# hdm0922/PathTracerDemo

Hardware: AMD Instinct MI355X
Metric: Msamples/sec at 1920x1080, 1 spp ReSTIR DI; per-pixel L2 vs WebGPU ref (higher is better)
Workload: dtype f32; 1 GPU; c3_interior_32 reuse 1920x1080, 1 spp/frame (configs[2]); frame=1920x1080, band_rows_per_gpu=1080, parallelism=row-bands x1

## Files before the change

pathtracerdemo_amd/csrc/ptx_api.cpp:

```cpp
#include <hip/hip_runtime.h>

#include <algorithm>
#include <cmath>
#include <cstdarg>
#include <cstdlib>
#include <cstdio>
#include <cstring>
#include <new>
#include <string>
#include <unordered_map>
#include <vector>

#include "ptx_internal.h"

namespace ptx {


[[maybe_unused]] static const char *const kShippedKnobs[] = {"COMM_TIMEOUT_S", "DEBUG_FILL", "HALO_PROXY_US"};
#if defined(PTX_WG_TIMES)
static const char *const kBuildKind = "wgt";
#elif defined(PTX_AB_BUILD)
static const char *const kBuildKind = "ab";
#else
static const char *const kBuildKind = "product";
// ... 439 lines not shown
                for (int k = 0; k < 3; ++k) P[v][k] = as_f32(G[vi + k]);
            }
            const float e1[3] = {P[1][0] - P[0][0], P[1][1] - P[0][1], P[1][2] - P[0][2]};
            const float e2[3] = {P[2][0] - P[0][0], P[2][1] - P[0][1], P[2][2] - P[0][2]};
            const float rec[12] = {P[0][0], P[0][1], P[0][2], e1[0], e1[1], e1[2], e2[0], e2[1], e2[2], 0, 0, 0};
            tris.insert(tris.end(), rec, rec + 12);
            float N[3][3];
            for (int v = 0; v < 3; ++v) {
                const size_t vi = (size_t)off_vertex + STRIDE_VERTEX * G[ii + v];
                if (vi + 6 > G.size()) return fail(h, PTX_E_SCENE, "vertex normal out of range");
                for (int k = 0; k < 3; ++k) N[v][k] = as_f32(G[vi + 3 + k]);
            }
            const float tv[20] = {P[0][0], P[0][1], P[0][2], N[0][0], N[0][1], N[0][2], P[1][0], P[1][1], P[1][2], N[1][0],
                                  N[1][1], N[1][2], P[2][0], P[2][1], P[2][2], N[2][0], N[2][1], N[2][2], 0.0f, 0.0f};
            tverts.insert(tverts.end(), tv, tv + 20);
        }
    }
    if (tris.empty()) tris.resize(12, 0.0f);
    if (tverts.empty()) tverts.resize(20, 0.0f);
    if (nodes.empty()) nodes.resize(1);
    if (subs.empty()) subs.resize(1);
    h->lay_subs = std::move(subs);
    h->lay_mat_word = std::move(mat_word);
    h->lay_mesh_sub_base = std::move(mesh_sub_base);
    h->lay_mesh_nsub = std::move(mesh_nsub);
    h->lay_mesh_tri_base = std::move(mesh_tri_base);
    h->lay_mesh_ntris = std::move(mesh_ntris);
    h->lay_mesh_vertex = std::move(mesh_vertex);
    h->lay_mesh_nverts = std::move(mesh_nverts);
    h->lay_mesh_node_base = std::move(mesh_node_base);
    h->lay_mesh_nnodes = std::move(mesh_nnodes);
    h->lay_mesh_levels = std::move(mesh_levels);
    h->lay_pair_words = std::move(pair_words);
    h->lay_root_word = std::move(root_word);
    if (int rc = upload(h, h->d_refit_order, order.data(), order.size() * sizeof(uint32_t))) return rc;
    {
        uint32_t most = 1;
        for (const uint32_t t : h->lay_mesh_ntris) most = std::max(most, t);
        if (int rc = alloc_buf(h, h->d_refit_box, (size_t)most * 6u * sizeof(float))) return rc;
    }
    h->n_inst = n_inst;
    if (int rc = layout_tables(h, true, true)) return rc;
    if (int rc = upload(h, h->d_tris, tris.data(), tris.size() * sizeof(float))) return rc;
    if (int rc = upload(h, h->d_nodes, nodes.data(), nodes.size() * sizeof(NodePair))) return rc;
    if (int rc = upload(h, h->d_tverts, tverts.data(), tverts.size() * sizeof(float))) return rc;
    h->n_tris = (uint32_t)(tris.size() / 12);
    h->n_nodes = (uint32_t)nodes.size();
    h->max_depth = max_depth;
    h->stack_depth = max_depth + 2u;
    if ((size_t)h->stack_depth * kBlock * 4u > 160u * 1024u)
        return fail(h, PTX_E_SCENE, "BLAS depth %u needs more LDS than a CU has", max_depth);
    h->layout_valid = true;
    h->layout_gen += 1u;
    for (auto &c : h->ctx) c.surf_valid = false;
    gbuf_key_drop_all(h);
    return PTX_OK;
}

Scene make_scene(ptx_handle *h) {
    Scene sc{};
    std::memcpy(sc.U, h->uniform, sizeof sc.U);
    sc.S = (const uint32_t *)h->d_scene.p;
    sc.G = (const uint32_t *)h->d_geometry.p;
    sc.tris = (const float4 *)h->d_tris.p;
    sc.nodes = (const NodePair *)h->d_nodes.p;
    sc.subs = (const SubRoot *)h->d_subs.p;
    sc.insts = (const Inst *)h->d_insts.p;
    sc.mats = (const float4 *)h->d_mats.p;
    sc.tverts = (const float4 *)h->d_tverts.p;
    sc.lights = sc.S ? sc.S + sc.U[U_OFF_LIGHT] : nullptr;
    sc.cdf = sc.S ? sc.S + sc.U[U_OFF_CDF] : nullptr;
    sc.n_inst = h->n_inst;
    sc.cull_box = h->cull_box;
    sc.cull_pad = h->cull_pad;
    sc.cull_scale = h->cull_scale;
    sc.n_subs = h->n_subs;
    sc.width = h->cfg.width;
    sc.height = h->cfg.height;
    sc.row_begin = h->cfg.row_begin;
    sc.row_end = h->cfg.row_end;
    sc.counters = (h->cfg.flags & PTX_FLAG_COUNT_WORK) ? (unsigned long long *)h->d_counters.p : nullptr;
    sc.census = (h->cfg.flags & PTX_FLAG_ROW_CENSUS) ? (unsigned long long *)h->d_census.p : nullptr;
    sc.frame_color = (float4 *)h->d_frame_color.p;
#ifdef PTX_WG_TIMES
    sc.wgt = (unsigned long long *)h->d_wgt.p;
#endif
    return sc;
}

void resolve_event(TimedLaunch &t, ptx_handle *h) {
    if (!t.pending) return;
    float ms = 0.0f;
    if (hipEventSynchronize(t.stop) == hipSuccess && hipEventElapsedTime(&ms, t.start, t.stop) == hipSuccess) {
        h->ms_total[t.pass] += ms;
        h->launches[t.pass] += 1;
    }
    t.pending = false;
}

static uint32_t seg_pixels(const ptx_handle *h) {
    static const uint32_t env_px = (uint32_t)ab_knob("SEG_PX", 0);
    if (env_px >= 256u && env_px <= 8192u && env_px % 256u == 0u) return env_px;
    const size_t npx = (size_t)h->band_h * h->cfg.width;
    if ((h->cfg.pipeline == PTX_PIPELINE_RESTIR && restir_pipe()) || (h->cfg.pipeline == PTX_PIPELINE_MCPT && mcpt_pipe()) ||
        h->cfg.pipeline == PTX_PIPELINE_RESTIR_GI) {
        const size_t p = (npx / 1152u + 128u) / 256u * 256u;
        return (uint32_t)std::min<size_t>(4096u, std::max<size_t>(kWaveSegPixels, p));
    }
    if (h->cfg.pipeline != PTX_PIPELINE_RESTIR_REUSE) return kWaveSegPixels;
    uint32_t p = 512u;
    while (p < 4096u && (size_t)(2u * p) * 1500u <= npx) p *= 2u;
    return p;
}

static size_t reuse_jobs_per_px(const ptx_handle *h) { return std::max<size_t>(2u * h->reuse_neighbors, kMotionJobs); }
int wave_buffers(ptx_handle *h, WaveBufs &w) {
    const size_t npix = (size_t)h->band_h * h->cfg.width;
    const uint32_t nl = h->uniform[U_LIGHT_COUNT];
    const size_t jpp = !has_reuse(h) ? 1u : h->cfg.pipeline == PTX_PIPELINE_RESTIR_GI ? 2u * h->reuse_neighbors
                                                                                         : reuse_jobs_per_px(h);
    const size_t per_px = std::max<size_t>(std::max<size_t>(2u, (size_t)nl + 1u), jpp);
    const size_t padded = (size_t)((h->cfg.width + 7u) / 8u) * ((h->band_h + 7u) / 8u) * 64u;
    const uint32_t seg_px = seg_pixels(h);
    const size_t nseg = (padded + seg_px - 1u) / seg_px;
    const size_t slots = nseg + 1u;
    const size_t cap = per_px * seg_px * slots;
    const size_t state_b = (size_t)kWaveStateSlots * npix * 16u, act_b = slots * seg_px * jpp * 4u;
    const size_t ctr_b = 2u * kWaveMaxRounds * slots * 4u;
    auto &c = h->cur();
    const bool resize = (c.wstate.p && c.wstate.bytes != state_b) || (c.wact[0].p && c.wact[0].bytes != act_b) ||
                        (c.wact[1].p && c.wact[1].bytes != act_b) || (c.wctr.p && c.wctr.bytes != ctr_b) ||
                        (c.wave_ray_cap && cap > c.wave_ray_cap);
    if (resize)
        if (int rc = quiesce(h)) return rc;
    if (int rc = alloc_buf(h, c.wstate, state_b)) return rc;
    if (int rc = alloc_buf(h, c.wact[0], act_b)) return rc;
    if (int rc = alloc_buf(h, c.wact[1], act_b)) return rc;
    const void *ctr_before = c.wctr.p;
    if (int rc = alloc_buf(h, c.wctr, ctr_b)) return rc;
    if (c.wctr.p != ctr_before) HIP_CHECK(h, memset_sync(h, c.wctr.p, 0, c.wctr.bytes));
    if (h->cfg.pipeline == PTX_PIPELINE_RESTIR_REUSE) {
        const size_t rp_b = slots * (1u + (size_t)seg_px) * 4u;
        if (h->d_replay.p && h->d_replay.bytes != rp_b && !resize)
            if (int rc = quiesce(h)) return rc;
        const void *rp_before = h->d_replay.p;
        if (int rc = alloc_buf(h, h->d_replay, rp_b)) return rc;
        if (h->d_replay.p != rp_before) HIP_CHECK(h, memset_sync(h, h->d_replay.p, 0, slots * 4u));
    }
    if (cap > c.wave_ray_cap) {
        free_buf(c.wrays);
        for (DevBuf &r : c.wres) free_buf(r);
        c.wave_ray_cap = 0;
        if (int rc = alloc_buf(h, c.wrays, cap * 32u)) return rc;
        for (int i = 0; i < (h->cfg.pipeline == PTX_PIPELINE_RESTIR_REUSE ? 3 : 2); ++i)
            if (int rc = alloc_buf(h, c.wres[i], cap * 32u)) return rc;
        c.wave_ray_cap = cap;
    }
    w.surf = nullptr;
    if (h->cfg.pipeline == PTX_PIPELINE_RESTIR_REUSE) {
        const size_t rows = (size_t)h->halo_top + h->band_h + h->halo_bot;
        if (c.surf.bytes != rows * h->cfg.width * 32u) c.surf_valid = false;
        if (int rc = alloc_buf(h, c.surf, rows * h->cfg.width * 32u)) return rc;
        w.surf = (uint4 *)c.surf.p + 2u * (size_t)h->halo_top * h->cfg.width;
    }
    w.state = (float4 *)c.wstate.p;
    w.npix = (uint32_t)npix;
    w.seg_px = seg_px;
    w.nseg = (uint32_t)nseg;
    w.ray_stride = (uint32_t)(per_px * seg_px);
    w.rays = (float4 *)c.wrays.p;
    for (int i = 0; i < 3; ++i) w.res[i] = (float4 *)c.wres[i].p;
    w.nres = 2;
    for (int i = 0; i < 2; ++i) w.act[i] = (uint32_t *)c.wact[i].p;
    w.act_stride = (uint32_t)(seg_px * jpp);
    w.cnt = (uint32_t *)c.wctr.p;
    w.seg_base = 0;
    w.seg_count = w.nseg;
    static const uint32_t cl = (uint32_t)ab_knob("SEG_CLUSTER", 1);
    w.cluster = (cl == 2u || cl == 4u || cl == 8u || cl == 16u) ? cl : 1u;
    if (h->cfg.flags & PTX_FLAG_ROW_CENSUS) w.cluster = seg_px / 64u;
    w.tile0 = 0;
    w.ntile0 = (uint32_t)(padded / 64u);
    w.tile1 = w.ntile1 = 0;
    w.seg_phys = 0;
    w.cnt_stride = (uint32_t)slots;
    return PTX_OK;
}

static TimedLaunch *event_begin(ptx_handle *h, int slot, hipStream_t st) {
    if (!(h->cfg.flags & PTX_FLAG_TIME_LAUNCHES)) return nullptr;
    TimedLaunch &t = h->ring[h->ring_pos];
    h->ring_pos = (h->ring_pos + 1) % kEventRing;
    resolve_event(t, h);
    if (hipEventRecord(t.start, st) != hipSuccess) return nullptr;
    t.pass = slot;
    return &t;
}
static void event_end(TimedLaunch *t, hipStream_t st) {
    if (t && hipEventRecord(t->stop, st) == hipSuccess) t->pending = true;
}

static size_t px_with_halo(const ptx_handle *h) {
    return (size_t)(h->halo_top + h->band_h + h->halo_bot) * h->cfg.width;
}
static uint32_t gi_job_slots(const ptx_handle *h) { return std::max(2u * h->reuse_neighbors, kGiMotionSlots); }
int reuse_buffers(ptx_handle *h) {
    const size_t njobs = (size_t)h->band_h * h->cfg.width *
                         (h->cfg.pipeline == PTX_PIPELINE_RESTIR_GI ? gi_job_slots(h) : reuse_jobs_per_px(h));
    if (h->cfg.pipeline == PTX_PIPELINE_RESTIR_GI) return alloc_buf(h, h->d_jres, njobs * 4u);
    if (int rc = alloc_buf(h, h->d_jstate, njobs * 6u * 16u)) return rc;
    if (int rc = alloc_buf(h, h->cur().nbr, px_with_halo(h) * 16u)) return rc;
    const size_t npix = (size_t)h->band_h * h->cfg.width;
    if (int rc = alloc_buf(h, h->cur().tjstate, npix * kMotionJobs * 6u * 16u)) return rc;
    if (int rc = alloc_buf(h, h->cur().tjres, npix * kMotionJobs * 16u)) return rc;
    return alloc_buf(h, h->d_jres, njobs * 16u);
}
static ReuseArgs reuse_args(ptx_handle *h, int pass) {
    ReuseArgs A{};
    A.gbuf = gbuf_band(h);
    A.cur = res_band(h);
    A.hist = hist_band(h);
    const bool temporal = pass == PTX_PASS_TEMPORAL;
    A.jstate = (float4 *)(temporal ? h->cur().tjstate.p : h->d_jstate.p);
    A.jres = (float4 *)(temporal ? h->cur().tjres.p : h->d_jres.p);
    A.jpp = temporal ? 1u : 2u * h->reuse_neighbors;
    A.njobs = h->band_h * h->cfg.width * A.jpp;
    static const bool planes = ab_knob("JOB_PLANES", 1) != 0;
    A.jpx = planes ? 1u : A.jpp;
    A.jslot = planes ? h->band_h * h->cfg.width : 1u;
    A.radius = h->reuse_radius;
    A.neighbors = h->reuse_neighbors;
    A.cap = h->temporal_cap;
    A.hist_valid = h->hist_valid && !h->hist_moved ? 1u : 0u;
    A.use_init = (pass == PTX_PASS_TEMPORAL && h->cur().init_state_valid) ? 1u : 0u;
    A.nbr_out = (uint4 *)h->cur().nbr.p + (size_t)h->halo_top * h->cfg.width;
    A.nbr = A.nbr_out;
    A.surf = h->cur().surf.p ? (const uint4 *)h->cur().surf.p + 2u * (size_t)h->halo_top * h->cfg.width : nullptr;
    static const bool fold_off = ab_knob("FOLD_LAST_STEP", 1) == 0;
    A.fold_last = ((pass == PTX_PASS_SPATIAL || pass == PTX_PASS_TEMPORAL) && !fold_off) ? 1u : 0u;
    A.ray_cap = (uint32_t)std::min<size_t>(h->cur().wave_ray_cap, 0xffffffffu);
    return A;
}

void mat4_inverse(const float *mf, float *out);
static ReuseArgs motion_args(ptx_handle *h) {
    ReuseArgs A = reuse_args(h, PTX_PASS_SPATIAL);
    A.jstate = (float4 *)h->cur().tjstate.p;
    A.jres = (float4 *)h->cur().tjres.p;
    A.jpp = kMotionJobs;
    A.njobs = h->band_h * h->cfg.width * A.jpp;
    static const bool planes = ab_knob("JOB_PLANES", 1) != 0;
    A.jpx = planes ? 1u : A.jpp;
    A.jslot = planes ? h->band_h * h->cfg.width : 1u;
    A.hist_valid = h->hist_valid ? 1u : 0u;
    A.use_init = h->cur().init_state_valid ? 1u : 0u;
    static const bool fold_on = ab_knob("FOLD_LAST_STEP", 1) != 0;
    A.fold_last = fold_on ? 1u : 0u;
    A.motion = 1u;
    std::memcpy(A.vpinv_prev, h->hist_camera, sizeof A.vpinv_prev);
    mat4_inverse(A.vpinv_prev, A.vp_prev);
    const size_t W = h->cfg.width;
    A.psurf = (const uint4 *)h->d_psurf.p + 2u * (size_t)h->halo_top * W;
    A.prev_row_lo = -(int32_t)h->halo_top;
    A.prev_row_hi = (int32_t)(h->band_h + h->halo_bot);
    A.clip = (unsigned long long *)h->d_counters.p + CNT_MOTION_CLIP;
    return A;
}

static GiArgs gi_args(ptx_handle *h, bool motion) {
    GiArgs A{};
    A.gbuf = gbuf_band(h);
    A.cur = res_band(h);
    A.hist = hist_band(h);
    A.direct = (float4 *)h->cur().direct.p;
    A.accum = (float4 *)h->d_accum.p;
    A.jray = (uint32_t *)h->d_jres.p;
    A.jpp = 2u * h->reuse_neighbors;
    static const bool planes = ab_knob("GI_JOB_PLANES", 1) != 0;
    A.jpx = planes ? 1u : A.jpp;
    A.jslot = planes ? h->band_h * h->cfg.width : 1u;
    if (!planes && motion) A.jpx = gi_job_slots(h);
    A.radius = h->reuse_radius;
    A.neighbors = h->reuse_neighbors;
    A.cap = h->temporal_cap;
    A.hist_valid = h->hist_valid && (motion || !h->hist_moved) ? 1u : 0u;
    if (motion) {
        std::memcpy(A.vpinv_prev, h->hist_camera, sizeof A.vpinv_prev);
        mat4_inverse(A.vpinv_prev, A.vp_prev);
        A.pgbuf = (const uint4 *)h->d_psurf.p + (size_t)h->halo_top * h->cfg.width;
        A.prev_row_lo = -(int32_t)h->halo_top;
        A.prev_row_hi = (int32_t)(h->band_h + h->halo_bot);
        A.clip = (unsigned long long *)h->d_counters.p + CNT_MOTION_CLIP;
    }
    return A;
}

static bool fuse_spatial_final(const ptx_handle *h, const Scene &sc, const int *passes, int npasses, int i) {
    static const bool on = ab_knob("FINAL_ONE", 1) != 0;
    return on && i + 1 < npasses && passes[i] == PTX_PASS_SPATIAL && passes[i + 1] == PTX_PASS_FINAL &&
           h->cfg.pipeline == PTX_PIPELINE_RESTIR_REUSE && tables_fit_lds(sc) && h->d_replay.p;
}

static hipError_t launch_wave_seq(ptx_handle *h, const Scene &sc, const WaveBufs &w, int pass, hipStream_t st,
                                  bool fused = false, hipEvent_t combine_after = nullptr,
                                  hipEvent_t combine_done = nullptr) {
    const uint4 *gb = gbuf_band(h);
    uint4 *res = res_band(h);
    float4 *acc = (float4 *)h->d_accum.p;
    hipError_t e = hipSuccess;
    if (h->cfg.pipeline == PTX_PIPELINE_RESTIR_GI) {
        const bool motion = is_motion_pass(pass);
        const GiArgs A = gi_args(h, motion);
        const int gp = motion ? 4 : pass == PTX_PASS_INIT ? 0 : pass == PTX_PASS_TEMPORAL ? 1 : pass == PTX_PASS_SPATIAL ? 2 : 3;
        const int rounds = gp == 0 ? kWaveRoundsGiInit : gp == 2 || gp == 4 ? kWaveRoundsGiSpatial : 0;
        for (int r = 0; e == hipSuccess && r <= rounds; ++r) {
            if (r > 0) {
                TimedLaunch *t = event_begin(h, PTX_STAT_WAVE_TRACE, st);
                e = wave_trace(sc, w, r - 1, 1, h->stack_depth, st, gp >= 2);
                event_end(t, st);
                if (e != hipSuccess) break;
            }
            TimedLaunch *t = event_begin(h, PTX_STAT_WAVE_LOGIC, st);
            e = wave_gi_round(sc, w, gp, r, A, st);
            event_end(t, st);
        }
        return e;
    }
    if (pass == PTX_PASS_TEMPORAL || pass == PTX_PASS_SPATIAL || pass == kPassTemporalJobs ||
        pass == kPassTemporalCombine || is_motion_pass(pass)) {
        const bool temporal = pass != PTX_PASS_SPATIAL;
        ReuseArgs A = is_motion_pass(pass) ? motion_args(h)
                                           : reuse_args(h, temporal ? PTX_PASS_TEMPORAL : PTX_PASS_SPATIAL);
        WaveBufs wj = w;
        if (A.fold_last && wj.res[2]) wj.nres = 3;
        else A.fold_last = 0u;
        if (fused && pass == PTX_PASS_SPATIAL) {
            A.fuse_final = 1u;
            A.accum = (float4 *)h->d_accum.p;
            A.replay_cnt = (uint32_t *)h->d_replay.p;
            A.replay = A.replay_cnt + w.cnt_stride;
            A.replay_total = (unsigned long long *)h->d_counters.p + CNT_REPLAY;
        }
        const int nr = reuse_rounds(temporal, A);
        const int r_first = pass == kPassTemporalCombine ? nr + 1 : 0;
        const int r_last = pass == kPassTemporalJobs ? nr : nr + 1;
        for (int r = r_first; e == hipSuccess && r <= r_last; ++r) {
            if (r > 0 && r <= nr) {
                TimedLaunch *t = event_begin(h, PTX_STAT_WAVE_TRACE, st);
                e = wave_trace(sc, wj, r - 1, 1, h->stack_depth, st);
                event_end(t, st);
            }
            if (e != hipSuccess) break;
            if (r == nr && A.fold_last) continue;
            const bool combine = r == nr + 1 && pass == PTX_PASS_SPATIAL;
            if (combine && combine_after && (e = hipStreamWaitEvent(st, combine_after, 0)) != hipSuccess) break;
            TimedLaunch *t = event_begin(h, PTX_STAT_WAVE_LOGIC, st);
            e = wave_reuse_round(sc, wj, temporal, r, A, st);
            event_end(t, st);
            if (combine && combine_done && e == hipSuccess) e = hipEventRecord(combine_done, st);
        }
        return e;
    }
    const uint4 *fres = h->cfg.pipeline == PTX_PIPELINE_RESTIR_REUSE ? (const uint4 *)hist_band(h) : res;
    static const bool final_one = ab_knob("FINAL_ONE", 1) != 0;
    if (pass == PTX_PASS_FINAL && final_one && h->cfg.pipeline == PTX_PIPELINE_RESTIR_REUSE && tables_fit_lds(sc)) {
        TimedLaunch *t = event_begin(h, PTX_STAT_WAVE_LOGIC, st);
        if (fused)
            e = wave_final_replay(sc, w, gb, fres, acc, (const uint32_t *)h->d_replay.p + w.cnt_stride,
                                  (uint32_t *)h->d_replay.p, h->stack_depth, st);
        else
            e = wave_final_one(sc, w, gb, fres, acc, h->stack_depth, st);
        event_end(t, st);
        h->launches[PTX_STAT_FINAL_FUSED] += 1;
        h->cur().init_state_valid = false;
        return e;
    }
    h->cur().init_state_valid = pass == PTX_PASS_INIT && h->cfg.pipeline == PTX_PIPELINE_RESTIR_REUSE;
    const int rounds = pass == PTX_PASS_INIT ? kWaveRoundsInit : pass == PTX_PASS_FINAL ? kWaveRoundsFinal
                                                                                        : kWaveRoundsMcpt;
    for (int r = 0; e == hipSuccess && r <= rounds; ++r) {
        if (r > 0) {
            TimedLaunch *t = event_begin(h, PTX_STAT_WAVE_TRACE, st);
            e = wave_trace(sc, w, r - 1, 1, h->stack_depth, st);
            event_end(t, st);
        }
        if (e != hipSuccess) break;
        TimedLaunch *t = event_begin(h, PTX_STAT_WAVE_LOGIC, st);
        e = pass == PTX_PASS_INIT    ? wave_init_round(sc, w, r, gb, res, st)
            : pass == PTX_PASS_FINAL ? wave_final_round(sc, w, r, gb, fres, acc, st)
                                     : wave_mcpt_round(sc, w, r, acc, h->mcpt_color, st);
        event_end(t, st);
    }
    return e;
}

hipError_t spatial_summaries(ptx_handle *h, hipStream_t st) {
    if (h->cfg.pipeline != PTX_PIPELINE_RESTIR_REUSE) return hipSuccess;
    const size_t W = h->cfg.width, top = h->halo_top * W, band = (size_t)h->band_h * W;
    const uint4 *gb = (const uint4 *)h->cur().gbuf.p, *rs = (const uint4 *)h->cur().res.p;
    uint4 *nb = (uint4 *)h->cur().nbr.p, *sf = (uint4 *)h->cur().surf.p;
    const Scene sc = make_scene(h);
    TimedLaunch *t = event_begin(h, PTX_STAT_WAVE_LOGIC, st);
    hipError_t e;
    if (!h->cur().nbr_valid) {
        e = wave_reuse_summary(sc, gb, rs, nb, sf, px_with_halo(h), st);
    } else {
        e = top ? wave_reuse_summary(sc, gb, rs, nb, sf, top, st) : hipSuccess;
        const size_t b0 = top + band;
        if (e == hipSuccess && px_with_halo(h) > b0)
            e = wave_reuse_summary(sc, gb + b0, rs + 8u * b0, nb + b0, sf ? sf + 2u * b0 : nullptr, px_with_halo(h) - b0,
                                   st);
    }
    event_end(t, st);
    return e;
}

static bool frames_in_flight(const ptx_handle *h) { return h->ctx[1].own && pipelined(h); }
static hipError_t fork_sequences(ptx_handle *h, int k) {
    auto &c = h->cur();
    hipError_t e = hipSuccess;
    if (k <= 1) return e;
    if (!c.ev_fork && (e = hipEventCreateWithFlags(&c.ev_fork, hipEventDisableTiming)) != hipSuccess) return e;
    for (int q = 1; q < k; ++q) {
        if (!c.sub[q] && (e = hipStreamCreateWithFlags(&c.sub[q], hipStreamNonBlocking)) != hipSuccess) return e;
        if (!c.ev_join[q] && (e = hipEventCreateWithFlags(&c.ev_join[q], hipEventDisableTiming)) != hipSuccess) return e;
    }
    if ((e = hipEventRecord(c.ev_fork, c.stream)) != hipSuccess) return e;
    for (int q = 1; q < k && e == hipSuccess; ++q) e = hipStreamWaitEvent(c.sub[q], c.ev_fork, 0);
    return e;
}
static hipError_t join_sequences(ptx_handle *h, int k) {
    auto &c = h->cur();
    hipError_t e = hipSuccess;
    for (int q = 1; q < k && e == hipSuccess; ++q)
        if ((e = hipEventRecord(c.ev_join[q], c.sub[q])) == hipSuccess) e = hipStreamWaitEvent(c.stream, c.ev_join[q], 0);
    return e;
}

static void seg_share(WaveBufs &part, uint32_t nseg, int q, int k) {
    part.seg_base = (uint32_t)((uint64_t)nseg * q / k);
    part.seg_count = (uint32_t)((uint64_t)nseg * (q + 1) / k) - part.seg_base;
}
static hipError_t spatial_overlap_seq(ptx_handle *h, const Scene &sc, const WaveBufs &interior, const WaveBufs &edge,
                                      hipEvent_t halo) {
    hipError_t e = hipSuccess;
    static const int env_bk = ab_knob("PIPE_BACK_STREAMS", 2);
    int k = env_bk > 0 && frames_in_flight(h) ? env_bk : 1;
    if (h->cfg.flags & PTX_FLAG_SINGLE_STREAM) k = 1;
    k = std::max(1, std::min<int>({k, ptx_handle::kMaxSplit, (int)interior.nseg, (int)edge.nseg}));
    ReuseArgs A = reuse_args(h, PTX_PASS_SPATIAL);
    const bool fold = A.fold_last && interior.res[2];
    if (!fold) A.fold_last = 0u;
    const int nr = reuse_rounds(0, A);
    if ((e = fork_sequences(h, k)) != hipSuccess) return e;
    const bool surf_stale = interior.surf && !h->cur().surf_valid;
    uint32_t E = 0u;
    for (int q = 0; q < k && e == hipSuccess; ++q) {
        hipStream_t st = q ? h->cur().sub[q] : h->cur().stream;
        WaveBufs wi = interior, we = edge;
        seg_share(wi, interior.nseg, q, k);
        seg_share(we, edge.nseg, q, k);
        wi.seg_phys = interior.seg_phys + E;
        we.seg_phys = interior.seg_phys + E + wi.seg_base + wi.seg_count - we.seg_base;
        E += we.seg_count;
        if (fold) wi.nres = we.nres = 3;
        WaveBufs wt = wi;
        wt.seg_count = wi.seg_count + we.seg_count;
        if (surf_stale) {
            if ((e = wave_surface(sc, wi, gbuf_band(h), st)) != hipSuccess) return e;
            if ((e = wave_surface(sc, we, gbuf_band(h), st)) != hipSuccess) return e;
        }
        for (int r = 0; e == hipSuccess && r <= nr + 1; ++r) {
            if (r > 0 && r <= nr) {
                TimedLaunch *t = event_begin(h, PTX_STAT_WAVE_TRACE, st);
                e = wave_trace(sc, wt, r - 1, 1, h->stack_depth, st);
                event_end(t, st);
                if (e != hipSuccess) break;
            }
            if (r == nr && A.fold_last) continue;
            TimedLaunch *t = event_begin(h, PTX_STAT_WAVE_LOGIC, st);
            e = wave_reuse_round(sc, wi, 0, r, A, st);
            if (e == hipSuccess && r == 0 && halo) e = hipStreamWaitEvent(st, halo, 0);
            if (e == hipSuccess) e = wave_reuse_round(sc, we, 0, r, A, st);
            event_end(t, st);
        }
        for (const WaveBufs *ws : {&wi, &we})
            if (e == hipSuccess) e = launch_wave_seq(h, sc, *ws, PTX_PASS_FINAL, st);
    }
    if (surf_stale && e == hipSuccess) h->cur().surf_valid = true;
    return e == hipSuccess ? join_sequences(h, k) : e;
}

hipError_t launch_wave_parts(ptx_handle *h, const Scene &sc, const WaveBufs &w, const int *passes, int npasses,
                             bool summaries, const WaveBufs *then, hipEvent_t then_wait, bool keep_gbuf) {
    h->hand_n = 0;
    static const bool overlap_start = ab_knob("OVERLAP_START", 1) != 0;
    if (then && overlap_start && npasses == 2 && passes[0] == PTX_PASS_SPATIAL && passes[1] == PTX_PASS_FINAL &&
        h->cfg.pipeline == PTX_PIPELINE_RESTIR_REUSE && !summaries)
        return spatial_overlap_seq(h, sc, w, *then, then_wait);
    static const int env_k = ab_knob("WAVE_STREAMS", 0);
    static const int env_pk = ab_knob("PIPE_STREAMS", 0);
    const bool band_h = h->comm || h->halo_top || h->halo_bot || (h->cfg.flags & PTX_FLAG_HALO_SKIP);
    const int pipe_k = env_pk > 0 ? env_pk : band_h || h->cfg.pipeline == PTX_PIPELINE_RESTIR_GI ? 1 : 2;
    int k = frames_in_flight(h) ? pipe_k : env_k > 0 ? env_k : 3;
    static const int env_bk = ab_knob("PIPE_BACK_STREAMS", 2);
    if (env_bk > 0 && frames_in_flight(h))
        for (int i = 0; i < npasses; ++i)
            if (passes[i] == PTX_PASS_SPATIAL) k = env_bk;
    if (h->cfg.flags & PTX_FLAG_SINGLE_STREAM) k = 1;
    k = std::max(1, std::min<int>(k, ptx_handle::kMaxSplit));
    if ((uint32_t)k > std::max(w.nseg, then ? then->nseg : 0u)) k = (int)std::max(w.nseg, then ? then->nseg : 0u);
    hipError_t e = hipSuccess;
    bool has_gbuf = false;
    for (int i = 0; i < npasses; ++i) has_gbuf |= passes[i] == PTX_PASS_GBUFFER;
    const bool skip_gbuf = has_gbuf && keep_gbuf && gbuf_kept(h);
    if (has_gbuf && !skip_gbuf) h->cur().gbuf_key_valid = false;
    for (int i = 0; i < npasses; ++i) {
        if (passes[i] == PTX_PASS_SPATIAL) {
            if (summaries && (e = spatial_summaries(h, h->cur().stream)) != hipSuccess) return e;
        } else if (passes[i] == PTX_PASS_GBUFFER && skip_gbuf) {
            continue;
        } else if (passes[i] != PTX_PASS_FINAL && passes[i] != PTX_PASS_TEMPORAL && passes[i] != kPassTemporalJobs &&
                   passes[i] != kPassTemporalCombine && !is_motion_pass(passes[i])) {
            h->cur().nbr_valid = false;
        }
    }
    bool need_surf[8] = {false};
    bool surf_ok = h->cur().surf_valid;
    for (int i = 0; i < npasses && i < 8; ++i) {
        if (passes[i] == PTX_PASS_GBUFFER) surf_ok = surf_ok && skip_gbuf;
        else if (passes[i] == PTX_PASS_INIT && w.surf) surf_ok = true;
        else if ((passes[i] == PTX_PASS_TEMPORAL || passes[i] == kPassTemporalJobs || passes[i] == PTX_PASS_SPATIAL ||
                  is_motion_pass(passes[i])) &&
                 w.surf) {
            need_surf[i] = !surf_ok;
            surf_ok = true;
        }
    }
    h->cur().surf_valid = surf_ok && w.surf;
    if (k == 0) return hipSuccess;
    if ((e = fork_sequences(h, k)) != hipSuccess) return e;
    for (int q = 0; q < k; ++q) {
        hipStream_t st = q ? h->cur().sub[q] : h->cur().stream;
        for (int set = 0; set < (then ? 2 : 1); ++set) {
            const WaveBufs &ws = set ? *then : w;
            if (set && then_wait && (e = hipStreamWaitEvent(st, then_wait, 0)) != hipSuccess) return e;
            WaveBufs part = ws;
            seg_share(part, ws.nseg, q, k);
            if (!part.seg_count) continue;
            for (int i = 0; i < npasses; ++i) {
                if (passes[i] == PTX_PASS_GBUFFER) {
                    if (skip_gbuf) continue;
                    TimedLaunch *t = event_begin(h, PTX_PASS_GBUFFER, st);
                    e = wave_gbuffer(sc, part, gbuf_band(h), h->stack_depth, st);
                    h->cur().init_state_valid = false;
                    event_end(t, st);
                } else {
                    if (i < 8 && need_surf[i]) {
                        TimedLaunch *t = event_begin(h, PTX_STAT_WAVE_LOGIC, st);
                        e = wave_surface(sc, part, gbuf_band(h), st);
                        event_end(t, st);
                        if (e != hipSuccess) return e;
                    }
                    const bool fused = !then && (fuse_spatial_final(h, sc, passes, npasses, i) ||
                                                 (i > 0 && fuse_spatial_final(h, sc, passes, npasses, i - 1)));
                    e = launch_wave_seq(h, sc, part, passes[i], st, fused);
                }
                if (e != hipSuccess) return e;
            }
        }
    }
    if ((e = join_sequences(h, k)) != hipSuccess) return e;
    if (has_gbuf && !skip_gbuf) {
        gbuf_key_of(h, h->cur().gbuf_key);
        h->cur().gbuf_key_valid = true;
    }
    for (int i = 0; i < npasses; ++i)
        if (passes[i] == PTX_PASS_TEMPORAL || passes[i] == kPassTemporalCombine || passes[i] == kPassTemporalMotion) {
            h->cur().init_state_valid = false;
            h->cur().nbr_valid = h->cfg.pipeline == PTX_PIPELINE_RESTIR_REUSE;
        }
    return hipSuccess;
}
static hipError_t launch_wave_pass(ptx_handle *h, const Scene &sc, const WaveBufs &w, int pass) {
    return launch_wave_parts(h, sc, w, &pass, 1);
}

static hipError_t launch_back_chain(ptx_handle *h, const Scene &sc, const WaveBufs &w, bool with_temporal,
                                    const hipEvent_t *hand, int n_hand) {
    auto &c = h->cur();
    if (h->comm || h->halo_top || h->halo_bot || (h->cfg.flags & PTX_FLAG_HALO_SKIP) || !w.surf || !c.surf_valid ||
        (!with_temporal && !c.nbr_valid))
        return hipErrorNotSupported;
    static const int env_bk = ab_knob("PIPE_BACK_STREAMS", 2);
    const int k = std::max(1, std::min<int>({env_bk > 0 ? env_bk : 1, ptx_handle::kMaxSplit, (int)w.nseg}));
    hipError_t e = hipSuccess;
    for (int q = 0; q < k; ++q) {
        if (!c.ev_tc[q] && (e = hipEventCreateWithFlags(&c.ev_tc[q], hipEventDisableTiming)) != hipSuccess) return e;
        if (!c.ev_hand[q] && (e = hipEventCreateWithFlags(&c.ev_hand[q], hipEventDisableTiming)) != hipSuccess) return e;
    }
    if ((e = fork_sequences(h, k)) != hipSuccess) return e;
    WaveBufs part[ptx_handle::kMaxSplit];
    for (int q = 0; q < k; ++q) {
        part[q] = w;
        seg_share(part[q], w.nseg, q, k);
    }
    for (int q = 0; q < k && with_temporal; ++q) {
        hipStream_t st = q ? c.sub[q] : c.stream;
        for (int i = 0; i < n_hand; ++i)
            if ((e = hipStreamWaitEvent(st, hand[i], 0)) != hipSuccess) return e;
        if (n_hand == 0 && (e = hipStreamWaitEvent(st, h->ev_prev, 0)) != hipSuccess) return e;
        if (part[q].seg_count && (e = launch_wave_seq(h, sc, part[q], kPassTemporalCombine, st)) != hipSuccess) return e;
        if ((e = hipEventRecord(c.ev_tc[q], st)) != hipSuccess) return e;
    }
    if (with_temporal) {
        c.init_state_valid = false;
        c.nbr_valid = true;
    }
// ... 1285 lines not shown
        reuse |= passes[i] == PTX_PASS_TEMPORAL || passes[i] == PTX_PASS_SPATIAL;
    }
    const uint32_t fl = h->cfg.flags;
    if (fl & (PTX_FLAG_SIMPLE_KERNELS | PTX_FLAG_COUNT_WORK)) {
        for (int i = 0; i < n; ++i)
            if (int rc = timed_launch(h, passes[i])) return rc;
        h->rendered = true;
        h->drawn |= gb;
        return PTX_OK;
    }
    if (!h->scene_loaded || !h->frame_set) return fail(h, PTX_E_INVALID, "scene and frame must be set before rendering");
    if (!h->layout_valid) {
        if (int rc = build_layout(h)) return rc;
    }
    Scene sc = make_scene(h);
    if (gb && !tables_fit_lds(sc)) {
        for (int i = 0; i < n; ++i)
            if (int rc = timed_launch(h, passes[i])) return rc;
        h->rendered = true;
        h->drawn |= gb;
        return PTX_OK;
    }
    WaveBufs w{};
    if (int rc = wave_buffers(h, w)) return rc;
    if (reuse)
        if (int rc = reuse_buffers(h)) return rc;
    TimedLaunch &t = h->ring[h->ring_pos];
    h->ring_pos = (h->ring_pos + 1) % kEventRing;
    resolve_event(t, h);
    HIP_CHECK(h, hipEventRecord(t.start, h->cur().stream));
    const hipError_t e = launch_wave_parts(h, sc, w, passes, n);
    if (e != hipSuccess) return fail(h, PTX_E_HIP, "ptx_run_passes: %s", hipGetErrorString(e));
    HIP_CHECK(h, hipEventRecord(t.stop, h->cur().stream));
    t.pass = PTX_STAT_PASS_GROUP;
    t.pending = true;
    for (int i = 0; i < n; ++i)
        if (passes[i] == PTX_PASS_SPATIAL) mark_history(h);
    h->rendered = true;
    h->drawn |= gb;
    return PTX_OK;
}

int ptx_halo_rows(ptx_handle *h, uint32_t *rows_top, uint32_t *rows_bottom, size_t *bytes_per_row) {
    if (!h) return PTX_E_INVALID;
    if (rows_top) *rows_top = h->halo_top;
    if (rows_bottom) *rows_bottom = h->halo_bot;
    if (bytes_per_row) *bytes_per_row = (size_t)h->cfg.width * (16u + 16u * h->res_u4);
    return PTX_OK;
}

static int halo_copy(ptx_handle *h, uint32_t r0, uint32_t rows, void *msg, bool to_msg) {
    if (!rows) return PTX_OK;
    const size_t W = h->cfg.width, rpx = 16u * h->res_u4, gb = rows * W * 16u, rb = rows * W * rpx;
    char *g = (char *)h->cur().gbuf.p + (size_t)r0 * W * 16u, *r = (char *)h->cur().res.p + (size_t)r0 * W * rpx;
    char *m = (char *)msg;
    if (to_msg) {
        HIP_CHECK(h, hipMemcpyAsync(m, g, gb, hipMemcpyDefault, h->cur().stream));
        HIP_CHECK(h, hipMemcpyAsync(m + gb, r, rb, hipMemcpyDefault, h->cur().stream));
    } else {
        gbuf_key_drop(h);
        HIP_CHECK(h, hipMemcpyAsync(g, m, gb, hipMemcpyDefault, h->cur().stream));
        HIP_CHECK(h, hipMemcpyAsync(r, m + gb, rb, hipMemcpyDefault, h->cur().stream));
    }
    return PTX_OK;
}

int ptx_halo_pack(ptx_handle *h, void *dev_top, void *dev_bottom) {
    if (!h) return PTX_E_INVALID;
    if ((h->halo_top && !dev_top) || (h->halo_bot && !dev_bottom)) return fail(h, PTX_E_INVALID, "ptx_halo_pack: null buffer");
    if (int rc = halo_copy(h, h->halo_top, h->halo_top, dev_top, true)) return rc;
    return halo_copy(h, h->halo_top + h->band_h - h->halo_bot, h->halo_bot, dev_bottom, true);
}

int ptx_halo_unpack(ptx_handle *h, const void *dev_top, const void *dev_bottom) {
    if (!h) return PTX_E_INVALID;
    if ((h->halo_top && !dev_top) || (h->halo_bot && !dev_bottom)) return fail(h, PTX_E_INVALID, "ptx_halo_unpack: null buffer");
    if (int rc = halo_copy(h, 0u, h->halo_top, (void *)dev_top, false)) return rc;
    return halo_copy(h, h->halo_top + h->band_h, h->halo_bot, (void *)dev_bottom, false);
}

int ptx_render(ptx_handle *h, float *rgba_out) {
    if (!h) return PTX_E_INVALID;
    HIP_CHECK(h, hipSetDevice(h->device));
    if (h->cfg.pipeline == PTX_PIPELINE_RESTIR) {
        int rc = timed_wave_frame(h);
        if (rc < 0) return rc;
        if (rc == 1)
            for (int p : {PTX_PASS_GBUFFER, PTX_PASS_INIT, PTX_PASS_FINAL})
                if ((rc = timed_launch(h, p))) return rc;
    } else if (has_reuse(h) && h->comm) {
        if (int rc = render_band_nccl(h)) return rc;
        if (rgba_out)
            if (int rc = read_to_host(h, rgba_out, h->d_accum.p, h->d_accum.bytes)) return rc;
        return PTX_OK;
    } else if (has_reuse(h) && (h->halo_top || h->halo_bot) && (h->cfg.flags & PTX_FLAG_HALO_SKIP)) {
        if (int rc = render_band_solo(h)) return rc;
        if (rgba_out)
            if (int rc = read_to_host(h, rgba_out, h->d_accum.p, h->d_accum.bytes)) return rc;
        return PTX_OK;
    } else if (has_reuse(h)) {
        if (h->halo_top || h->halo_bot)
            return fail(h, PTX_E_INVALID, "a band of the reuse pipeline renders with a communicator "
                                          "(ptx_comm_init), through ptx_render_bands, or ptx_run_passes + ptx_halo_*");
        int rc = timed_wave_frame(h);
        if (rc < 0) return rc;
        if (rc == 1)
            for (int p : {PTX_PASS_GBUFFER, PTX_PASS_INIT, PTX_PASS_TEMPORAL, PTX_PASS_SPATIAL, PTX_PASS_FINAL})
                if ((rc = timed_launch(h, p))) return rc;
    } else if (pipelined(h)) {
        int rc = timed_wave_frame(h);
        if (rc < 0) return rc;
        if (rc == 1 && (rc = timed_launch(h, PTX_PASS_MCPT))) return rc;
    } else {
        if (int rc = timed_launch(h, PTX_PASS_MCPT)) return rc;
    }
    h->frames++;
    h->rendered = h->drawn = true;
    if (rgba_out)
        if (int rc = read_to_host(h, rgba_out, h->d_accum.p, h->d_accum.bytes)) return rc;
    return PTX_OK;
}

int ptx_reset_accumulation(ptx_handle *h) {
    if (!h) return PTX_E_INVALID;
    HIP_CHECK(h, hipMemsetAsync(h->d_accum.p, 0, h->d_accum.bytes, h->cur().stream));
    h->hist_valid = false;
    h->dn_hist_valid = false;
    h->ut_valid = false;
    return PTX_OK;
}

int ptx_synchronize(ptx_handle *h) {
    if (!h) return PTX_E_INVALID;
    HIP_CHECK(h, hipStreamSynchronize(h->cur().stream));
    return PTX_OK;
}

int ptx_get_stats(ptx_handle *h, ptx_stats *out) {
    if (!h || !out) return PTX_E_INVALID;
    for (auto &t : h->ring) resolve_event(t, h);
    std::memset(out, 0, sizeof *out);
    out->frames = h->frames;
    for (int p = 0; p < kPasses; ++p) {
        out->kernel_ms_total[p] = h->ms_total[p];
        out->kernel_launches[p] = h->launches[p];
    }
    out->triangles = h->n_tris;
    out->bvh_nodes = h->n_nodes;
    out->instances = h->n_inst;
    out->max_bvh_depth = h->max_depth;
    const auto &c = h->cur();
    out->device_bytes = h->d_scene.bytes + h->d_geometry.bytes + h->d_tris.bytes + h->d_nodes.bytes + h->d_subs.bytes +
                        h->d_insts.bytes + h->d_mats.bytes + h->d_tverts.bytes + c.gbuf.bytes + c.res.bytes + h->d_accum.bytes +
                        h->d_hist.bytes + h->d_jstate.bytes + h->d_jres.bytes + c.tjstate.bytes + c.tjres.bytes + c.nbr.bytes +
                        c.surf.bytes + h->d_psurf.bytes + c.direct.bytes + h->d_dn_guide.bytes + h->d_dn_work.bytes +
                        h->d_denoised.bytes + h->d_frame_color.bytes + h->d_dn_guide_prev.bytes + h->d_dn_hist[0].bytes +
                        h->d_dn_hist[1].bytes + h->d_dn_mom[0].bytes + h->d_dn_mom[1].bytes + h->d_dn_halo_g.bytes +
                        h->d_dn_halo_c.bytes + h->d_dn_obj.bytes + h->d_dn_snap.bytes + h->d_up_halo.bytes + h->d_ut_guide[0].bytes + h->d_ut_guide[1].bytes +
                        h->d_ut_hist[0].bytes + h->d_ut_hist[1].bytes + h->d_refit_order.bytes + h->d_refit_box.bytes;
    for (const auto &k : h->skins) out->device_bytes += k.bind.bytes + k.target_pos.bytes + k.target_nrm.bytes + k.pose.bytes;
    return PTX_OK;
}

int ptx_reset_stats(ptx_handle *h) {
    if (!h) return PTX_E_INVALID;
    for (auto &t : h->ring) t.pending = false;
    HIP_CHECK(h, hipStreamSynchronize(h->cur().stream));
    for (int p = 0; p < kPasses; ++p) { h->ms_total[p] = 0.0; h->launches[p] = 0; }
    h->frames = 0;
    HIP_CHECK(h, memset_sync(h, h->d_counters.p, 0, h->d_counters.bytes));
    if (h->d_census.p) HIP_CHECK(h, memset_sync(h, h->d_census.p, 0, h->d_census.bytes));
    return PTX_OK;
}

#ifdef PTX_WG_TIMES
int ptx_diag_wave_times(ptx_handle *h, uint64_t *out, size_t max_records) {
    if (!h || !h->d_wgt.p) return PTX_E_INVALID;
    HIP_CHECK(h, hipDeviceSynchronize());
    uint64_t n = 0;
    HIP_CHECK(h, copy_sync(h, &n, h->d_wgt.p, 8, hipMemcpyDeviceToHost));
    n = std::min<uint64_t>(std::min<uint64_t>(n, 1u << 20), max_records);
    if (n && out) HIP_CHECK(h, copy_sync(h, out, (uint64_t *)h->d_wgt.p + 4, n * 32u, hipMemcpyDeviceToHost));
    HIP_CHECK(h, memset_sync(h, h->d_wgt.p, 0, 8));
    return (int)n;
}
#endif

int ptx_row_census(ptx_handle *h, uint64_t *out, size_t n_tile_rows) {
    if (!h || !out) return PTX_E_INVALID;
    if (!(h->cfg.flags & PTX_FLAG_ROW_CENSUS)) return fail(h, PTX_E_INVALID, "handle has no PTX_FLAG_ROW_CENSUS");
    const uint32_t tile_rows = (h->band_h + 7u) / 8u, tiles_x = (h->cfg.width + 7u) / 8u;
    if (n_tile_rows != tile_rows) return fail(h, PTX_E_INVALID, "census: %zu tile rows, band has %u", n_tile_rows, tile_rows);
    std::vector<unsigned long long> c((size_t)h->census_blocks * kCensusWords);
    HIP_CHECK(h, copy_sync(h, c.data(), h->d_census.p, c.size() * 8u, hipMemcpyDeviceToHost));
    std::memset(out, 0, (size_t)tile_rows * 5u * sizeof(uint64_t));
    for (uint32_t r = 0; r < tile_rows; ++r)
        for (int k = 0; k < 5; ++k) out[5u * r + k] += c[(size_t)kCensusWords * r + k];
    const uint32_t m = seg_pixels(h) / 64u, ntiles = tile_rows * tiles_x;
    for (uint32_t s = 0; tile_rows + s < h->census_blocks && (size_t)s * m < ntiles; ++s) {
        const unsigned long long *b = c.data() + (size_t)kCensusWords * (tile_rows + s);
        const uint32_t t0 = s * m, t1 = std::min(ntiles, t0 + m), r0 = t0 / tiles_x, r1 = (t1 - 1u) / tiles_x;
        for (int k = 0; k < 5; ++k) {
            uint64_t left = b[k];
            for (uint32_t r = r0; r <= r1; ++r) {
                const uint32_t a = std::max(t0, r * tiles_x), z = std::min(t1, (r + 1u) * tiles_x);
                const uint64_t part = r == r1 ? left : b[k] * (z - a) / (t1 - t0);
                out[5u * r + k] += part;
                left -= part;
            }
        }
    }
    return PTX_OK;
}

int ptx_read_buffer(ptx_handle *h, int which, void *host_dst, size_t bytes) {
    if (!h || !host_dst) return PTX_E_INVALID;
    DevBuf b;
    if (!buffer_view(h, which, b) || bytes > b.bytes)
        return fail(h, PTX_E_INVALID, "read of %zu bytes from buffer %d", bytes, which);
    if (int rc = read_to_host(h, host_dst, b.p, bytes)) return rc;
    return PTX_OK;
}

int ptx_write_buffer(ptx_handle *h, int which, const void *host_src, size_t bytes) {
    if (!h || !host_src) return PTX_E_INVALID;
    DevBuf b;
    if (which == PTX_BUF_DENOISED) return fail(h, PTX_E_INVALID, "the denoised image is ptx_denoise's output: read-only");
    if (which == PTX_BUF_FRAME_COLOR || which == PTX_BUF_DENOISE_HISTORY)
        return fail(h, PTX_E_INVALID, "buffer %d is the renderer's / ptx_denoise's output: read-only", which);
    if (which == PTX_BUF_UPSAMPLE_HISTORY)
        return fail(h, PTX_E_INVALID, "buffer %d is ptx_upsample_temporal's output: read-only", which);
    if (!buffer_view(h, which, b) || bytes > b.bytes)
        return fail(h, PTX_E_INVALID, "write of %zu bytes to buffer %d", bytes, which);
    HIP_CHECK(h, copy_sync(h, b.p, host_src, bytes, hipMemcpyHostToDevice));
    h->cur().init_state_valid = false;
    h->cur().nbr_valid = false;
    h->cur().surf_valid = false;
    if (which == PTX_BUF_GBUFFER) gbuf_key_drop(h);
    return PTX_OK;
}

int ptx_device_pointer(ptx_handle *h, int which, void **dev_ptr, size_t *bytes) {
    if (!h || !dev_ptr) return PTX_E_INVALID;
    DevBuf b;
    if (!buffer_view(h, which, b)) return fail(h, PTX_E_INVALID, "unknown buffer %d", which);
    *dev_ptr = b.p;
    if (bytes) *bytes = b.bytes;
    if (which == PTX_BUF_GBUFFER) {
        h->gbuf_exposed = true;
        gbuf_key_drop_all(h);
    }
    return PTX_OK;
}

int ptx_present(ptx_handle *h, uint32_t canvas_w, uint32_t canvas_h, int bgra, uint8_t *out) {
    if (!h || !out) return PTX_E_INVALID;
    if (canvas_w == 0 || canvas_h == 0 || (uint64_t)canvas_w * canvas_h > (1ull << 28))
        return fail(h, PTX_E_INVALID, "ptx_present: canvas %ux%u", canvas_w, canvas_h);
    if (h->cfg.row_begin != 0 || h->band_h != h->cfg.height)
        return fail(h, PTX_E_INVALID, "ptx_present: a band handle (rows %u..%u) holds part of the texture: present the "
                                      "gathered frame on the host", h->cfg.row_begin, h->cfg.row_end);
    if (!h->d_accum.p) return fail(h, PTX_E_INVALID, "ptx_present: nothing rendered");
    HIP_CHECK(h, hipSetDevice(h->device));
    const size_t bytes = (size_t)canvas_w * canvas_h * 4u;
    if (int rc = alloc_buf(h, h->d_canvas, bytes)) return rc;
    const hipError_t e = launch_present(present_texture(h), h->cfg.width, h->cfg.height, canvas_w, canvas_h,
                                        bgra != 0, (uint32_t *)h->d_canvas.p, h->cur().stream);
    if (e != hipSuccess) return fail(h, PTX_E_HIP, "ptx_present: %s", hipGetErrorString(e));
    return read_to_host(h, out, h->d_canvas.p, bytes);
}

int ptx_present_async(ptx_handle *h, uint32_t canvas_w, uint32_t canvas_h, int bgra) {
    if (!h) return PTX_E_INVALID;
    if (h->present_pending) return fail(h, PTX_E_INVALID, "ptx_present_async: a present is in flight (poll it first)");
    if (canvas_w == 0 || canvas_h == 0 || (uint64_t)canvas_w * canvas_h > (1ull << 28))
        return fail(h, PTX_E_INVALID, "ptx_present_async: canvas %ux%u", canvas_w, canvas_h);
    if (h->cfg.row_begin != 0 || h->band_h != h->cfg.height)
        return fail(h, PTX_E_INVALID, "ptx_present_async: a band handle holds part of the texture");
    if (!h->d_accum.p) return fail(h, PTX_E_INVALID, "ptx_present_async: nothing rendered");
    HIP_CHECK(h, hipSetDevice(h->device));
    const size_t bytes = (size_t)canvas_w * canvas_h * 4u;
    if (int rc = alloc_buf(h, h->d_canvas_async, bytes)) return rc;
    if (bytes > h->present_host_bytes) {
        if (h->present_host) (void)hipHostFree(h->present_host);
        h->present_host = nullptr;
        h->present_host_bytes = 0;
        HIP_CHECK(h, hipHostMalloc(&h->present_host, bytes, hipHostMallocDefault));
        h->present_host_bytes = bytes;
    }
    if (!h->ev_present) HIP_CHECK(h, hipEventCreateWithFlags(&h->ev_present, hipEventDisableTiming));
    const hipError_t e = launch_present(present_texture(h), h->cfg.width, h->cfg.height, canvas_w, canvas_h,
                                        bgra != 0, (uint32_t *)h->d_canvas_async.p, h->cur().stream);
    if (e != hipSuccess) return fail(h, PTX_E_HIP, "ptx_present_async: %s", hipGetErrorString(e));
    HIP_CHECK(h, hipMemcpyAsync(h->present_host, h->d_canvas_async.p, bytes, hipMemcpyDeviceToHost, h->cur().stream));
    HIP_CHECK(h, hipEventRecord(h->ev_present, h->cur().stream));
    h->present_bytes = bytes;
    h->present_pending = true;
    return PTX_OK;
}

int ptx_present_poll(ptx_handle *h, uint8_t *out, size_t bytes) {
    if (!h || !out) return PTX_E_INVALID;
    if (!h->present_pending) return fail(h, PTX_E_INVALID, "ptx_present_poll: no present in flight");
    if (bytes < h->present_bytes)
        return fail(h, PTX_E_INVALID, "ptx_present_poll: %zu bytes; the canvas needs %zu", bytes, h->present_bytes);
    const hipError_t e = hipEventQuery(h->ev_present);
    if (e == hipErrorNotReady) return PTX_E_PENDING;
// ... 24 lines not shown
int ptx_upsample(ptx_handle *hi, ptx_handle *lo, const ptx_upsample_params *p) {
    if (!hi || !lo) return PTX_E_INVALID;
    const char *what = "ptx_upsample";
    if (hi == lo) return fail(hi, PTX_E_INVALID, "%s: one handle on both sides", what);
    float sigma_plane;
    if (int rc = upsample_params(hi, p, sigma_plane, what)) return rc;
    for (ptx_handle *h : {hi, lo})
        if (h->cfg.row_begin != 0 || h->band_h != h->cfg.height)
            return fail(hi, PTX_E_INVALID, "%s: the %s handle is a band (rows %u..%u): ptx_upsample_bands", what,
                        h == hi ? "full-size" : "small", h->cfg.row_begin, h->cfg.row_end);
    uint32_t s = 0;
    if (int rc = upsample_pair_check(hi, hi, lo, s, what)) return rc;
    HIP_CHECK(hi, hipSetDevice(hi->device));
    if (int rc = upsample_alloc(hi, 0u, lo->cfg.width)) return rc;
    if (int rc = upsample_source(hi, lo)) return rc;
    HIP_CHECK(hi, hipStreamWaitEvent(hi->cur().stream, lo->ev_up_src, 0));
    const hipError_t e = upsample_launch(hi, lo, s, sigma_plane, 0u, 0u);
    if (int rc = upsample_done(hi, hi)) return rc;
    if (int rc = upsample_release(hi, lo, hi)) return rc;
    if (e != hipSuccess) return fail(hi, PTX_E_HIP, "%s launch: %s", what, hipGetErrorString(e));
    return PTX_OK;
}

int ptx_phase_uniform(const uint32_t hi_uniform[PTX_UNIFORM_WORDS], uint32_t s, uint32_t px, uint32_t py,
                      uint32_t lo_uniform_out[PTX_UNIFORM_WORDS]) {
    if (!hi_uniform || !lo_uniform_out) return PTX_E_INVALID;
    if (s < 2u || s > 4u || px >= s || py >= s) return PTX_E_INVALID;
    const uint32_t W = hi_uniform[0], H = hi_uniform[1];
    if (W == 0u || H == 0u || W % s != 0u || H % s != 0u) return PTX_E_INVALID;
    uint32_t u[PTX_UNIFORM_WORDS];
    std::memcpy(u, hi_uniform, sizeof u);
    u[0] = W / s;
    u[1] = H / s;
    const float dx = (float)(2 * (int)px - ((int)s - 1)) / (float)W, dy = (float)(2 * (int)py - ((int)s - 1)) / (float)H;
    if (dx != 0.0f || dy != 0.0f) {
#pragma clang fp contract(off)
        float m[16];
        std::memcpy(m, u + 4, sizeof m);
        for (int k = 0; k < 4; ++k) {
            const float a = dx * m[k], b = dy * m[4 + k];
            const float t = m[12 + k] + a;
            m[12 + k] = t + b;
        }
        std::memcpy(u + 4, m, sizeof m);
    }
    std::memcpy(lo_uniform_out, u, sizeof u);
    return PTX_OK;
}

int ptx_upsample_temporal(ptx_handle *hi, ptx_handle *lo, const ptx_upsample_temporal_params *p) {
    if (!hi || !lo) return PTX_E_INVALID;
    const char *what = "ptx_upsample_temporal";
    if (hi == lo) return fail(hi, PTX_E_INVALID, "%s: one handle on both sides", what);
    UtCall c;
    if (int rc = upsample_temporal_params(hi, p, c, what, false)) return rc;
    for (ptx_handle *h : {hi, lo})
        if (h->cfg.row_begin != 0 || h->band_h != h->cfg.height)
            return fail(hi, PTX_E_INVALID, "%s: the %s handle is a band (rows %u..%u): bands are not supported by this call", what,
                        h == hi ? "full-size" : "small", h->cfg.row_begin, h->cfg.row_end);
    uint32_t s = 0;
    if (int rc = upsample_pair_check(hi, hi, lo, s, what, false)) return rc;
    if (int rc = upsample_temporal_camera(hi, hi, lo, s, c, what)) return rc;
    HIP_CHECK(hi, hipSetDevice(hi->device));
    if (int rc = upsample_temporal_alloc(hi, hi, 0u, lo->cfg.width)) return rc;
    if (int rc = upsample_source(hi, lo)) return rc;
    HIP_CHECK(hi, hipStreamWaitEvent(hi->cur().stream, lo->ev_up_src, 0));
    const hipError_t e = upsample_temporal_launch(hi, lo, s, c, 0u, 0u, 0u, 0u);
    if (int rc = upsample_done(hi, hi)) return rc;
    if (int rc = upsample_release(hi, lo, hi)) return rc;
    if (e != hipSuccess) return fail(hi, PTX_E_HIP, "%s launch: %s", what, hipGetErrorString(e));
    return PTX_OK;
}

int ptx_present_source(ptx_handle *h, int which) {
    if (!h) return PTX_E_INVALID;
    if (which != PTX_BUF_ACCUM && which != PTX_BUF_DENOISED)
        return fail(h, PTX_E_INVALID, "ptx_present_source: buffer %d (PTX_BUF_ACCUM or PTX_BUF_DENOISED)", which);
    if (which == PTX_BUF_DENOISED && !h->d_denoised.p)
        return fail(h, PTX_E_INVALID, "ptx_present_source: no denoised image yet (ptx_denoise first)");
    h->present_src = which;
    return PTX_OK;
}

int ptx_trace_device(ptx_handle *h, const void *rays_dev, void *hits_dev, size_t n, int eps_mode) {
    if (!h || (n && (!rays_dev || !hits_dev)) || n > 0xffffffffu || (eps_mode != 0 && eps_mode != 1))
        return fail(h, PTX_E_INVALID, "ptx_trace: bad arguments");
    if (!h->scene_loaded || !h->frame_set) return fail(h, PTX_E_INVALID, "scene and frame must be set before tracing");
    if (!h->layout_valid) {
        if (int rc = build_layout(h)) return rc;
    }
    TimedLaunch &t = h->ring[h->ring_pos];
    h->ring_pos = (h->ring_pos + 1) % kEventRing;
    resolve_event(t, h);
    Scene sc = make_scene(h);
    HIP_CHECK(h, hipEventRecord(t.start, h->cur().stream));
    const bool simple = (h->cfg.flags & PTX_FLAG_SIMPLE_KERNELS) != 0;
    hipError_t e = (simple ? launch_trace_rays : launch_trace_rays_sm)(
        sc, (const float4 *)rays_dev, (float4 *)hits_dev, (uint32_t)n, eps_mode, h->stack_depth, h->cur().stream);
    if (e != hipSuccess) return fail(h, PTX_E_HIP, "trace launch: %s", hipGetErrorString(e));
    HIP_CHECK(h, hipEventRecord(t.stop, h->cur().stream));
    t.pass = PTX_PASS_TRACE;
    t.pending = true;
    return PTX_OK;
}

int ptx_trace(ptx_handle *h, const float *rays, float *hits, size_t n, int eps_mode) {
    if (!h || (n && (!rays || !hits))) return fail(h, PTX_E_INVALID, "ptx_trace: null arrays");
    if (n == 0) return PTX_OK;
    if (int rc = alloc_buf(h, h->d_qrays, std::max(h->d_qrays.bytes, n * 32u))) return rc;
    if (int rc = alloc_buf(h, h->d_qhits, std::max(h->d_qhits.bytes, n * 32u))) return rc;
    HIP_CHECK(h, hipMemcpyAsync(h->d_qrays.p, rays, n * 32u, hipMemcpyHostToDevice, h->cur().stream));
    if (int rc = ptx_trace_device(h, h->d_qrays.p, h->d_qhits.p, n, eps_mode)) return rc;
    return read_to_host(h, hits, h->d_qhits.p, n * 32u);
}

int ptx_trace_queries(ptx_handle *h, const float *queries, float *results, size_t n, int eps_mode, int occ_only) {
    if (!h || (n && (!queries || !results))) return fail(h, PTX_E_INVALID, "ptx_trace_queries: null arrays");
    if (eps_mode != 0 && eps_mode != 1) return fail(h, PTX_E_INVALID, "ptx_trace_queries: eps_mode %d (0 or 1)", eps_mode);
    if (h->cfg.flags & (PTX_FLAG_SIMPLE_KERNELS | PTX_FLAG_ROW_CENSUS))
        return fail(h, PTX_E_INVALID, "ptx_trace_queries: the handle has no wavefront trace kernel of its own "
                                      "(PTX_FLAG_SIMPLE_KERNELS) or maps queue slots to tile rows (PTX_FLAG_ROW_CENSUS)");
    if (!h->scene_loaded || !h->frame_set) return fail(h, PTX_E_INVALID, "scene and frame must be set before tracing");
    if (n > 0x7fffffffu) return fail(h, PTX_E_INVALID, "ptx_trace_queries: %zu queries (32-bit ray slots)", n);
    for (size_t i = 0; i < n; ++i) {
        uint32_t kind;
        std::memcpy(&kind, queries + 8u * i + 7u, sizeof kind);
        if (kind > 2u) return fail(h, PTX_E_INVALID, "ptx_trace_queries: query %zu has kind %u (0 closest, 1 Visibility, 2 occlusion)", i, kind);
        if (occ_only && kind != 2u)
            return fail(h, PTX_E_INVALID, "ptx_trace_queries: occ_only with query %zu of kind %u (every query must be 2, occlusion)", i, kind);
    }
    if (n == 0) return PTX_OK;
    if (!h->layout_valid) {
        if (int rc = build_layout(h)) return rc;
    }
    const uint32_t nseg = (uint32_t)((n + kWaveSegPixels - 1u) / kWaveSegPixels);
    const size_t slots = (size_t)nseg * kWaveSegPixels;
    std::vector<uint32_t> cnt(2u * (size_t)nseg, 0u);
    for (uint32_t j = 0; j < nseg; ++j)
        cnt[nseg + j] = (uint32_t)std::min<size_t>(kWaveSegPixels, n - (size_t)j * kWaveSegPixels);
    if (int rc = alloc_buf(h, h->d_qrays, std::max(h->d_qrays.bytes, slots * 32u))) return rc;
    if (int rc = alloc_buf(h, h->d_qhits, std::max(h->d_qhits.bytes, slots * 32u))) return rc;
    if (int rc = alloc_buf(h, h->d_qcnt, std::max(h->d_qcnt.bytes, cnt.size() * 4u))) return rc;
    hipStream_t st = h->cur().stream;
    HIP_CHECK(h, hipMemcpyAsync(h->d_qrays.p, queries, n * 32u, hipMemcpyHostToDevice, st));
    HIP_CHECK(h, hipMemcpyAsync(h->d_qcnt.p, cnt.data(), cnt.size() * 4u, hipMemcpyHostToDevice, st));
    HIP_CHECK(h, hipMemsetAsync(h->d_qhits.p, 0, n * 32u, st));
    WaveBufs w{};
    w.seg_px = kWaveSegPixels;
    w.nseg = w.seg_count = w.cnt_stride = nseg;
    w.cluster = 1;
    w.ray_stride = kWaveSegPixels;
    w.rays = (float4 *)h->d_qrays.p;
    w.res[0] = w.res[1] = (float4 *)h->d_qhits.p;
    w.nres = 2;
    w.cnt = (uint32_t *)h->d_qcnt.p;
    TimedLaunch &t = h->ring[h->ring_pos];
    h->ring_pos = (h->ring_pos + 1) % kEventRing;
    resolve_event(t, h);
    Scene sc = make_scene(h);
    HIP_CHECK(h, hipEventRecord(t.start, st));
    hipError_t e = wave_trace(sc, w, 0, eps_mode, h->stack_depth, st, occ_only != 0);
    if (e != hipSuccess) return fail(h, PTX_E_HIP, "trace launch: %s", hipGetErrorString(e));
    HIP_CHECK(h, hipEventRecord(t.stop, st));
    t.pass = PTX_PASS_TRACE;
    t.pending = true;
    return read_to_host(h, results, h->d_qhits.p, n * 32u);
}

int ptx_set_stream(ptx_handle *h, void *hip_stream) {
    if (!h) return PTX_E_INVALID;
    if (int rc = first_frame_ctx(h)) return rc;
    if (h->ev_up_src || h->d_denoised.p)
        if (int rc = quiesce(h)) return rc;
    h->ctx[0].stream = hip_stream ? (hipStream_t)hip_stream : h->ctx[0].own;
    h->dn_stream = h->ctx[0].stream;
    gbuf_key_drop_all(h);
    return PTX_OK;
}

int ptx_destroy(ptx_handle *h) {
    if (!h) return PTX_E_INVALID;
    (void)hipSetDevice(h->device);
    (void)quiesce(h);
    if (h->xstream) (void)hipStreamSynchronize(h->xstream);
    comm_destroy(h);
    if (h->ctx[0].own) (void)hipStreamSynchronize(h->ctx[0].own);
    for (auto &t : h->ring) {
        if (t.start) (void)hipEventDestroy(t.start);
        if (t.stop) (void)hipEventDestroy(t.stop);
    }
    if (h->host_stage) (void)hipHostFree(h->host_stage);
    if (h->ev_present) {
        (void)hipEventSynchronize(h->ev_present);
        (void)hipEventDestroy(h->ev_present);
    }
    if (h->present_host) (void)hipHostFree(h->present_host);
    for (DevBuf *b : {&h->d_canvas, &h->d_canvas_async, &h->d_scene, &h->d_geometry, &h->d_tris, &h->d_nodes, &h->d_subs,
                      &h->d_insts, &h->d_mats, &h->d_tverts, &h->d_accum, &h->d_counters, &h->d_qrays, &h->d_qhits, &h->d_qcnt, &h->d_hist,
                      &h->d_jstate, &h->d_jres, &h->d_replay, &h->d_psurf, &h->d_census, &h->d_wgt, &h->d_dn_guide, &h->d_dn_work,
                      &h->d_denoised, &h->d_frame_color, &h->d_dn_guide_prev, &h->d_dn_hist[0], &h->d_dn_hist[1], &h->d_dn_mom[0],
                      &h->d_dn_mom[1], &h->d_dn_halo_g, &h->d_dn_halo_c, &h->d_dn_obj, &h->d_dn_snap, &h->d_up_halo, &h->d_ut_guide[0], &h->d_ut_guide[1],
                      &h->d_ut_hist[0], &h->d_ut_hist[1], &h->d_refit_order, &h->d_refit_box})
        free_buf(*b);
    drop_skins(h);
    for (auto &c : h->ctx) {
        for (DevBuf *b : {&c.gbuf, &c.res, &c.direct, &c.nbr, &c.tjstate, &c.tjres, &c.surf, &c.wstate, &c.wrays, &c.wres[0],
                          &c.wres[1], &c.wres[2], &c.wact[0], &c.wact[1], &c.wctr})
            free_buf(*b);
        if (c.ev_fork) (void)hipEventDestroy(c.ev_fork);
        for (int q = 0; q < ptx_handle::kMaxSplit; ++q) {
            if (c.ev_join[q]) (void)hipEventDestroy(c.ev_join[q]);
            if (c.sub[q]) (void)hipStreamDestroy(c.sub[q]);
        }
        if (c.own) (void)hipStreamDestroy(c.own);
    }
    if (h->ev_prev) (void)hipEventDestroy(h->ev_prev);
    if (h->ev_dn_ready) (void)hipEventDestroy(h->ev_dn_ready);
    if (h->ev_dn_copied) (void)hipEventDestroy(h->ev_dn_copied);
    if (h->ev_up_src) (void)hipEventDestroy(h->ev_up_src);
    if (h->ev_up_done) (void)hipEventDestroy(h->ev_up_done);
    if (h->ev_ut_ready) (void)hipEventDestroy(h->ev_ut_ready);
    if (h->ev_ut_copied) (void)hipEventDestroy(h->ev_ut_copied);
    delete h;
    return PTX_OK;
}

const char *ptx_last_error(const ptx_handle *h) { return h ? h->err.c_str() : "null handle"; }

}
```

pathtracerdemo_amd/csrc/ptx_internal.h:

```cpp
#pragma once
#include <hip/hip_runtime.h>

#include <algorithm>
#include <string>

#include "../../include/ptx.h"
#include "ptx_launch.h"

namespace ptx {
constexpr int kPasses = 16;
constexpr int kEventRing = 256;
struct DevBuf {
    void *p = nullptr;
    size_t bytes = 0;
};
struct TimedLaunch {
    hipEvent_t start = nullptr, stop = nullptr;
    int pass = -1;
    bool pending = false;
};
}

using namespace ptx;

constexpr int kPassTemporalJobs = 0x100, kPassTemporalCombine = 0x101;
constexpr int kPassTemporalMotion = 0x102;
inline bool is_motion_pass(int p) {
    return p == kPassTemporalMotion;
}

constexpr uint8_t kStaleGeometry = 1u, kStaleAccel = 2u;

struct ptx_handle {
    ptx_config cfg{};
    int device = 0;
    std::string err;

    std::vector<uint32_t> scene, geometry, accel;
    DevBuf d_scene, d_geometry;
    DevBuf d_tris, d_nodes, d_subs, d_insts, d_mats, d_tverts;
    uint32_t n_tris = 0, n_nodes = 0, n_inst = 0, n_subs = 0, max_depth = 0, stack_depth = 0;
    float cull_box = 0.0f, cull_pad = 0.0f, cull_scale = 0.0f;
    uint32_t layout_key[8] = {0};
    bool layout_valid = false;
    std::vector<SubRoot> lay_subs;
    std::vector<size_t> lay_mat_word;
    std::vector<uint32_t> lay_mesh_sub_base, lay_mesh_nsub, lay_mesh_tri_base;
    std::vector<uint32_t> lay_mesh_ntris, lay_mesh_vertex, lay_mesh_nverts, lay_mesh_node_base, lay_mesh_nnodes;
    std::vector<std::vector<uint32_t>> lay_mesh_levels;
    std::vector<uint32_t> lay_pair_words, lay_root_word;
    DevBuf d_refit_order, d_refit_box;
    struct Skin {
        uint32_t first = 0, n = 0, n_joints = 0, n_targets = 0;
        double w_max = 0.0, p_max = 0.0, d_max = 0.0;
        DevBuf bind, target_pos, target_nrm, pose;
    };
    std::vector<Skin> skins;
    std::vector<uint8_t> mesh_stale;
    bool scene_loaded = false;
    uint32_t uniform[PTX_UNIFORM_WORDS] = {0};
    bool frame_set = false;
    uint32_t band_h = 0, halo_top = 0, halo_bot = 0;
    DevBuf d_accum, d_counters, d_hist, d_jstate, d_jres;
    DevBuf d_replay;
    uint32_t res_u4 = 8;
    bool gbuf_exposed = false;
    uint32_t reuse_radius = 0, reuse_neighbors = 0, temporal_cap = 0;
    float4 *mcpt_color = nullptr;
    bool hist_valid = false;
    uint32_t hist_camera[19] = {0};
    bool hist_moved = false;
    bool hist_same_only = false;
    DevBuf d_psurf;
    DevBuf d_qrays, d_qhits;
    DevBuf d_qcnt;
    DevBuf d_census;
    uint32_t census_blocks = 0;
    DevBuf d_wgt;
    static constexpr int kMaxCtx = 3;
    static constexpr int kMaxSplit = 4;
    static constexpr int kGbufKeyWords = 32;
    struct FrameCtx {
        DevBuf gbuf, res, direct;
        DevBuf nbr, tjstate, tjres;
        DevBuf surf;
        DevBuf wstate, wrays, wres[3], wact[2], wctr;
        size_t wave_ray_cap = 0;
        hipStream_t own = nullptr, stream = nullptr;
        hipStream_t sub[kMaxSplit] = {nullptr, nullptr, nullptr, nullptr};
        hipEvent_t ev_fork = nullptr, ev_join[kMaxSplit] = {nullptr, nullptr, nullptr, nullptr};
        hipEvent_t ev_tc[kMaxSplit] = {nullptr, nullptr, nullptr, nullptr};
        hipEvent_t ev_hand[kMaxSplit] = {nullptr, nullptr, nullptr, nullptr};
        bool init_state_valid = false;
        bool nbr_valid = false;
        bool surf_valid = false;
        uint32_t gbuf_key[kGbufKeyWords] = {0};
        bool gbuf_key_valid = false;
    } ctx[kMaxCtx];
    int ctx_idx = 0;
    FrameCtx &cur() { return ctx[ctx_idx]; }
    const FrameCtx &cur() const { return ctx[ctx_idx]; }
    hipEvent_t ev_prev = nullptr;
    int hand_ctx = 0, hand_n = 0;
    void *comm = nullptr;
    int rank = 0, world = 1;
    hipStream_t xstream = nullptr;
    hipEvent_t ev_front = nullptr, ev_halo = nullptr;
    hipEvent_t ev_mhalo = nullptr;
    uint64_t halo_bytes_sent = 0;
    bool comm_broken = false;
    uint64_t band_frames = 0;
    uint32_t band_camera[19] = {0};
    DevBuf d_canvas;
    void *host_stage = nullptr;
    size_t host_stage_bytes = 0;
    DevBuf d_canvas_async;
    void *present_host = nullptr;
    size_t present_host_bytes = 0, present_bytes = 0;
    hipEvent_t ev_present = nullptr;
    bool present_pending = false;
    DevBuf d_dn_guide, d_dn_work, d_denoised;
    DevBuf d_frame_color;
    DevBuf d_dn_guide_prev, d_dn_hist[2], d_dn_mom[2];
    int dn_set = 0;
    bool dn_hist_valid = false;
    uint32_t dn_camera[19] = {0};
    float dn_vp[16] = {0};
    std::vector<uint32_t> dn_insts;
    DevBuf d_dn_obj;
    bool dn_track = false;
    uint32_t dn_track_layout = 0, layout_gen = 0;
    DevBuf d_dn_snap;
    std::vector<uint8_t> dn_deformed;
    uint32_t dn_cap_top = 0, dn_cap_bot = 0;
    DevBuf d_dn_halo_g, d_dn_halo_c;
    uint32_t dn_cov_lo = 0, dn_cov_hi = 0;
    hipEvent_t ev_dn_ready = nullptr, ev_dn_copied = nullptr;
    bool dn_guide_swapped = false, drawn = false;
    hipStream_t dn_stream = nullptr;
    hipEvent_t ev_up_src = nullptr, ev_up_done = nullptr;
    uint32_t dn_guide_top = 0, dn_guide_bot = 0;
    DevBuf d_up_halo;
    DevBuf d_ut_guide[2], d_ut_hist[2];
    int ut_set = 0;
    bool ut_valid = false, dn_guide_stale = false;
    uint32_t ut_camera[19] = {0};
    float ut_vp[16] = {0};
    hipEvent_t ev_ut_ready = nullptr, ev_ut_copied = nullptr;
    uint32_t nb_rows[2][2] = {{0, 0}, {0, 0}};
    int present_src = PTX_BUF_ACCUM;
    bool rendered = false;
    TimedLaunch ring[kEventRing];
    int ring_pos = 0;
    double ms_total[kPasses] = {};
    uint64_t launches[kPasses] = {};
    uint64_t frames = 0;
};

namespace ptx {
int fail(ptx_handle *h, int code, const char *fmt, ...);
#define HIP_CHECK(h, expr)                                                                                   \
    do {                                                                                                     \
        hipError_t e_ = (expr);                                                                              \
        if (e_ != hipSuccess) return fail((h), PTX_E_HIP, "%s: %s (%s:%d)", #expr, hipGetErrorString(e_),      \
                                          __FILE__, __LINE__);                                               \
    } while (0)
void free_buf(DevBuf &b);
int alloc_buf(ptx_handle *h, DevBuf &b, size_t bytes);
int read_to_host(ptx_handle *h, void *dst, const void *src, size_t bytes);
uint4 *gbuf_band(ptx_handle *h);
uint4 *res_band(ptx_handle *h);
bool has_reuse(const ptx_handle *h);
int build_layout(ptx_handle *h);
Scene make_scene(ptx_handle *h);
void resolve_event(TimedLaunch &t, ptx_handle *h);
int wave_buffers(ptx_handle *h, WaveBufs &w);
int reuse_buffers(ptx_handle *h);
hipError_t launch_wave_parts(ptx_handle *h, const Scene &sc, const WaveBufs &w, const int *passes, int npasses,
                             bool summaries = true, const WaveBufs *then = nullptr, hipEvent_t then_wait = nullptr,
                             bool keep_gbuf = false);
void gbuf_key_of(const ptx_handle *h, uint32_t *key);
void gbuf_key_drop(ptx_handle *h);
void gbuf_key_drop_all(ptx_handle *h);
hipError_t spatial_summaries(ptx_handle *h, hipStream_t st);
void mark_history(ptx_handle *h);
int motion_prepare(ptx_handle *h, hipStream_t st);
uint4 *hist_band(ptx_handle *h);
bool pipelined(const ptx_handle *h);
int quiesce(ptx_handle *h);
int pipe_depth();
int ensure_contexts(ptx_handle *h);
void next_frame_ctx(ptx_handle *h);
int first_frame_ctx(ptx_handle *h);
struct DnCall {
    uint32_t n = 5, temporal = 0, follow = 0;
    float sigma_lum = 4.0f, sigma_plane = 0.02f, alpha_min = 0.05f;
};
struct DnBand {
    uint32_t top = 0, bot = 0;
    int wr = 0;
};
inline uint32_t dn_reach(uint32_t n) { return 2u << n; }
int denoise_params(ptx_handle *h, const ptx_denoise_params *p, DnCall &c, const char *what);
int denoise_check(ptx_handle *h, const DnCall &c, const char *what);
int denoise_alloc(ptx_handle *h, const DnCall &c);
int denoise_front(ptx_handle *h, const DnCall &c, DnBand &b);
int denoise_back(ptx_handle *h, const DnCall &c, const DnBand &b);
int upsample_params(ptx_handle *err, const ptx_upsample_params *p, float &sigma_plane, const char *what);
int upsample_pair_check(ptx_handle *err, ptx_handle *hi, ptx_handle *lo, uint32_t &s, const char *what, bool same_camera = true);
int upsample_alloc(ptx_handle *hi, uint32_t halo_rows, uint32_t w);
int upsample_source(ptx_handle *err, ptx_handle *lo);
hipError_t upsample_launch(ptx_handle *hi, ptx_handle *lo, uint32_t s, float sigma_plane, uint32_t top, uint32_t bot);
int upsample_done(ptx_handle *err, ptx_handle *hi);
int upsample_release(ptx_handle *err, ptx_handle *lo, ptx_handle *hi);
constexpr uint32_t kUtRowsDefault = 32, kUtRowsMax = 128;
struct UtCall {
    float sigma_plane = 0.02f, alpha_min = 0.02f, alpha_fill = 0.05f;
    uint32_t px = 0, py = 0, rows = kUtRowsDefault;
};
inline uint32_t ut_cap_top(const ptx_handle *h) { return std::min(kUtRowsMax, h->cfg.row_begin); }
inline uint32_t ut_cap_bot(const ptx_handle *h) { return std::min(kUtRowsMax, h->cfg.height - h->cfg.row_end); }
int upsample_temporal_params(ptx_handle *err, const ptx_upsample_temporal_params *p, UtCall &c, const char *what, bool bands);
int upsample_temporal_camera(ptx_handle *err, ptx_handle *hi, ptx_handle *lo, uint32_t s, const UtCall &c, const char *what);
int upsample_temporal_alloc(ptx_handle *err, ptx_handle *hi, uint32_t halo_rows, uint32_t w);
hipError_t upsample_temporal_launch(ptx_handle *hi, ptx_handle *lo, uint32_t s, const UtCall &c, uint32_t top, uint32_t bot,
                                    uint32_t ht, uint32_t hb);
int render_band_nccl(ptx_handle *h);
int render_band_solo(ptx_handle *h);
void comm_destroy(ptx_handle *h);
const char *comm_library();
}
```

pathtracerdemo_amd/csrc/ptx_launch.h:

```cpp
#pragma once

#include <hip/hip_runtime.h>

#include "ptx_device.h"

namespace ptx {

constexpr int kTile = 16;
constexpr int kBlock = 256;

int env_knob(const char *key, int dflt);
#ifdef PTX_AB_BUILD
inline int ab_knob(const char *key, int dflt) { return env_knob(key, dflt); }
#else
constexpr int ab_knob(const char *, int dflt) { return dflt; }
#endif

enum : int { SL_INIT_START = 1, SL_INIT_STEP = 2, SL_TEMPORAL_START = 4, SL_JOB_STEP = 16 };
inline bool shade_from_lds(const Scene &sc, int kernel_bit) {
    static const int mask = ab_knob("SHADE_LDS", SL_INIT_START | SL_INIT_STEP | SL_TEMPORAL_START | SL_JOB_STEP);
    return shading_fits_lds(sc) && (mask & kernel_bit) != 0;
}
inline size_t shade_lds_bytes(bool staged, const Scene &sc) { return staged ? shading_lds_bytes(sc) : 0u; }

inline size_t stack_lds_bytes(uint32_t depth) { return (size_t)depth * kBlock * sizeof(uint32_t); }

hipError_t launch_gbuffer(const Scene &sc, uint4 *gbuf, uint32_t stack_depth, hipStream_t s);
hipError_t launch_init(const Scene &sc, const uint4 *gbuf, uint4 *reservoir, uint32_t stack_depth, hipStream_t s);
hipError_t launch_final(const Scene &sc, const uint4 *gbuf, const uint4 *reservoir, float4 *accum,
                        uint32_t stack_depth, hipStream_t s);
hipError_t launch_mcpt(const Scene &sc, float4 *accum, uint32_t stack_depth, hipStream_t s);
hipError_t launch_present(const float4 *tex, uint32_t W, uint32_t H, uint32_t cw, uint32_t ch, bool bgra,
                          uint32_t *out, hipStream_t s);

struct DnWin {
    uint32_t y0;
    uint32_t rows;
    uint32_t c0, c1;
};
struct DnImage {
    const float4 *own, *halo;
    uint32_t o0, o1;
};
hipError_t launch_denoise_guide(const Scene &sc, const uint4 *gbuf, float4 *guide, float sigma_plane, hipStream_t s);
hipError_t launch_denoise_guide_halo(const Scene &sc, const uint4 *texels, uint32_t top, uint32_t bottom, float4 *guide,
                                     float sigma_plane, hipStream_t s);
hipError_t launch_denoise_variance(uint32_t W, const DnWin &win, const DnImage &img, const float4 *guide, float4 *out,
                                   hipStream_t s);
hipError_t launch_denoise_atrous(uint32_t W, const DnWin &win, uint32_t step, const float4 *in, const float4 *guide,
                                 float4 *out, float sigma_lum, bool last, hipStream_t s);
struct DnObj {
    float d[16];
    uint32_t flag;
    uint32_t pad[3];
};
struct DnPrev {
    float m[16], minv[16];
    uint32_t mesh, tri_base;
    uint32_t pad[2];
};
struct DnVerts {
    const uint4 *gbuf = nullptr;
    const DnPrev *prev = nullptr;
    const float4 *snap = nullptr;
};
hipError_t launch_denoise_temporal(uint32_t W, uint32_t H, const DnWin &win, const float *vp_prev, float alpha_min,
                                   uint32_t mode, uint32_t prev_y0, uint32_t prev_rows, const float4 *guide,
                                   const float4 *frame, const float4 *accum, const float4 *pguide, const float4 *phist,
                                   const float2 *pmom, float4 *hist, float2 *mom, unsigned long long *clip,
                                   const DnObj *obj, uint32_t n_obj, const DnVerts &verts, hipStream_t s);
hipError_t launch_denoise_variance_moments(uint32_t W, const DnWin &win, const float4 *hist, const float2 *mom,
                                           const float4 *guide, float4 *out, hipStream_t s);
hipError_t launch_denoise_upsample(uint32_t s, uint32_t W, uint32_t H, const float4 *guide_hi, const float4 *guide_lo,
                                   const float4 *color_lo, float4 *out, hipStream_t st);
hipError_t launch_denoise_upsample_temporal(uint32_t s, uint32_t W, uint32_t H, uint32_t px, uint32_t py, float alpha_min,
                                            float alpha_fill, uint32_t mode, const float *vp_prev, const float4 *guide_hi,
                                            const float4 *guide_lo, const float4 *color_lo, const float4 *guide_prev,
                                            const float4 *hist_prev, float4 *hist, float4 *out, hipStream_t st);
struct UpWin {
    uint32_t y0, rows, o0, o1;
    uint32_t Y0, Y1;
};
hipError_t launch_denoise_upsample_win(uint32_t s, uint32_t W, uint32_t H, const UpWin &win, const float4 *guide_hi,
                                       const float4 *guide_lo, const float4 *color_lo, const float4 *halo_lo, float4 *out,
                                       hipStream_t st);
struct UtWin {
    UpWin up;
    uint32_t hy0, hrows;
    unsigned long long *clip;
};
hipError_t launch_denoise_upsample_temporal_win(uint32_t s, uint32_t W, uint32_t H, uint32_t px, uint32_t py, float alpha_min,
                                                float alpha_fill, uint32_t mode, const float *vp_prev, const UtWin &win,
                                                const float4 *guide_hi, const float4 *guide_lo, const float4 *color_lo,
                                                const float4 *halo_lo, const float4 *guide_prev, const float4 *hist_prev,
                                                float4 *hist, float4 *out, hipStream_t st);

struct RefitMesh {
    const uint32_t *G;
    float4 *tris, *tverts;
    NodePair *nodes;
    SubRoot *subs;
    float2 *box;
    const uint32_t *order;
    uint32_t vertex, index;
    uint32_t tri_base, n_tris, sub_base, n_subs;
};
hipError_t launch_refit_tris(const RefitMesh &m, hipStream_t s);
hipError_t launch_refit_level(const RefitMesh &m, uint32_t first, uint32_t n, hipStream_t s);
hipError_t launch_refit_roots(const RefitMesh &m, hipStream_t s);

constexpr uint32_t kSkinMaxJoints = 256u, kSkinMaxTargets = 8u;
struct SkinArgs {
    uint32_t *G;
    const float4 *bind;
    const float *target_pos, *target_nrm;
    const float4 *palette;
    const float *target_weights;
    uint32_t word0, n, n_joints, n_targets;
};
hipError_t launch_skin_vertices(const SkinArgs &a, hipStream_t s);

hipError_t launch_trace_rays(const Scene &sc, const float4 *rays, float4 *hits, uint32_t n, int eps_mode,
                             uint32_t stack_depth, hipStream_t s);

constexpr uint32_t kWaveStateSlots = 10u;
constexpr uint32_t kStateCs2 = 7u, kStateCs3 = 8u, kStateTsel = 9u;
constexpr uint32_t kWaveSegPixels = 768u;
constexpr int kWaveRoundsInit = 3, kWaveRoundsFinal = 3, kWaveRoundsMcpt = 4;
constexpr int kWaveMaxRounds = 5;
struct WaveBufs {
    float4 *state;
    uint32_t npix;
    uint32_t seg_px;
    uint32_t nseg;
    uint32_t seg_base;
    uint32_t seg_count;
    uint32_t cluster;
    uint32_t ray_stride;
    float4 *rays;
    float4 *res[3];
    uint32_t nres;
    uint32_t *act[2];
    uint32_t act_stride;
    uint32_t *cnt;
    uint32_t tile0, ntile0, tile1, ntile1;
    uint32_t seg_phys, cnt_stride;
    uint4 *surf;
};
hipError_t wave_trace(const Scene &sc, const WaveBufs &w, int round, int eps_mode, uint32_t stack_depth,
                      hipStream_t s, bool occ_only = false);
hipError_t wave_init_round(const Scene &sc, const WaveBufs &w, int round, const uint4 *gbuf, uint4 *reservoir,
                           hipStream_t s);
hipError_t wave_final_one(const Scene &sc, const WaveBufs &w, const uint4 *gbuf, const uint4 *reservoir, float4 *accum,
                          uint32_t depth, hipStream_t s);
hipError_t wave_final_replay(const Scene &sc, const WaveBufs &w, const uint4 *gbuf, const uint4 *reservoir, float4 *accum,
                             const uint32_t *replay, uint32_t *replay_cnt, uint32_t depth, hipStream_t s);
hipError_t wave_final_round(const Scene &sc, const WaveBufs &w, int round, const uint4 *gbuf, const uint4 *reservoir,
                            float4 *accum, hipStream_t s);
hipError_t wave_gbuffer(const Scene &sc, const WaveBufs &w, uint4 *gbuf, uint32_t stack_depth, hipStream_t s);
hipError_t launch_trace_rays_sm(const Scene &sc, const float4 *rays, float4 *hits, uint32_t n, int eps_mode,
                                uint32_t stack_depth, hipStream_t s);
hipError_t wave_mcpt_round(const Scene &sc, const WaveBufs &w, int round, float4 *accum, float4 *color,
                           hipStream_t s);
hipError_t wave_mix_frame(const Scene &sc, const float4 *color, float4 *accum, hipStream_t s);

constexpr int kWaveRoundsReuse = 3;
struct ReuseArgs {
    const uint4 *gbuf;
    uint4 *cur;
    uint4 *hist;
    float4 *jstate;
    float4 *jres;
    uint32_t njobs, jpp;
    uint32_t jpx, jslot;
    uint32_t radius, neighbors, cap, hist_valid;
    uint32_t use_init;
    const uint4 *nbr;
    uint4 *nbr_out;
    const uint4 *surf;
    uint32_t fold_last;
    uint32_t ray_cap;
    uint32_t motion;
    float vpinv_prev[16], vp_prev[16];
    const uint4 *psurf;
    int32_t prev_row_lo, prev_row_hi;
    unsigned long long *clip;
    uint32_t fuse_final;
    float4 *accum;
    uint32_t *replay, *replay_cnt;
    unsigned long long *replay_total;
};
constexpr uint32_t kMotionJobs = 3u;
constexpr uint32_t kJobPending = 0xFFFFFFFFu;
static_assert(kWaveRoundsReuse <= 3, "fold_last: one result buffer per reuse trace round");
int reuse_rounds(int pass_temporal, const ReuseArgs &A);
hipError_t wave_reuse_round(const Scene &sc, const WaveBufs &w, int pass_temporal, int round, const ReuseArgs &A,
                            hipStream_t s);
hipError_t wave_reuse_summary(const Scene &sc, const uint4 *gbuf, const uint4 *res, uint4 *nbr, uint4 *surf,
                              size_t npx, hipStream_t s);
hipError_t wave_surface(const Scene &sc, const WaveBufs &w, const uint4 *gbuf, hipStream_t s);

constexpr int kWaveRoundsGiInit = 2, kWaveRoundsGiSpatial = 1;
constexpr uint32_t kGiResU4 = 4u;
struct GiArgs {
    const uint4 *gbuf;
    uint4 *cur;
    uint4 *hist;
    float4 *direct;
    float4 *accum;
    uint32_t *jray;
    uint32_t jpp;
    uint32_t jpx, jslot;
    uint32_t radius, neighbors, cap, hist_valid;
    float vpinv_prev[16], vp_prev[16];
    const uint4 *pgbuf;
    int32_t prev_row_lo, prev_row_hi;
    unsigned long long *clip;
};
constexpr uint32_t kGiMotionSlots = 4u;
hipError_t wave_gi_round(const Scene &sc, const WaveBufs &w, int pass, int round, const GiArgs &A, hipStream_t s);

}
```

pathtracerdemo_amd/csrc/ptx_reuse.hip:

```cpp
#include "ptx_wave_common.h"

namespace ptx {

constexpr uint32_t SALT_TEMPORAL = 0x54454D50u, SALT_SPATIAL = 0x53504154u;

enum : uint32_t { JS_HDR, JS_F, JS_CUR, JS_NRM, JS_PREV, JS_RRF, JS_COUNT };
constexpr uint32_t kJobFresh = 1u << 24;
constexpr uint32_t kResReuseLayout = 0x100u;
#ifndef PTX_JOB_FRESH
#define PTX_JOB_FRESH 1
#endif

struct Job {
    uint32_t i, length, phase, seed1, idx, matref;
    uint32_t k, lab;
    bool shift, rok;
    int32_t ref;
    int32_t dom;
    f3 f;
    float prod;
    Surface cur;
    f3 prev;
    float beta, rr_p;
    f3 rr_f;
// ... 61 lines not shown
        prev = x0_of(sc, (uint32_t)(dom - q * W), (uint32_t)((int32_t)sc.row_begin + q));
    } else if (s.phase != 1u) {
        const float4 cu = st[JS_CUR * n + jid], nr = st[JS_NRM * n + jid];
        const float4 pv = st[JS_PREV * n + jid], rf = st[JS_RRF * n + jid];
        matref = asu(cu.w);
        cur.pos = mk(cu.x, cu.y, cu.z);
        cur.nrm = mk(nr.x, nr.y, nr.z);
        cur.mat = material_at(sc, matref);
        beta = nr.w;
        prev = mk(pv.x, pv.y, pv.z); rr_p = pv.w;
        rr_f = mk(rf.x, rf.y, rf.z);
    }
    s.seed1 = seed1; s.matref = matref; s.dom = dom;
    s.f = f; s.rr_f = rr_f; s.prev = prev;
    s.beta = beta; s.rr_p = rr_p;
    s.cur = cur;
}

__device__ __forceinline__ bool rr_step(Job &s, const Surface &X, f3 L, f3 fv, float pdf) {
    s.rr_f = s.rr_f * (fv * fabsf(dot(X.nrm, L)));
    s.rr_p *= pdf;
    const float ps = luminance(s.rr_f) / s.rr_p;
    const bool ok = ps > 0.0f;
    s.rr_p *= ps;
    if (ps > 1.0f) s.beta /= ps;
    return ok;
}

__device__ __forceinline__ void job_init(Job &s, f3 x0, const Surface &X1, uint32_t matref, int32_t ref,
                                         uint32_t length, uint32_t seed1, int32_t dom, uint32_t k, bool shift) {
    s.i = 1u; s.length = length; s.phase = 0u; s.seed1 = seed1; s.idx = 0u; s.ref = ref; s.dom = dom;
    s.k = min(k, 7u); s.lab = 0u; s.shift = shift; s.rok = false;
    s.f = mk(1.0f, 1.0f, 1.0f); s.prod = 1.0f;
    s.prev = x0;
    s.cur = X1;
    s.matref = matref;
    s.beta = 1.0f; s.rr_p = 1.0f; s.rr_f = mk(1.0f, 1.0f, 1.0f);
}
__device__ __forceinline__ bool job_begin(const Scene &sc, const ReuseArgs &A, Job &s, uint32_t x, uint32_t y,
                                          int32_t dom, int32_t ref) {
    const uint4 *rv = res_at(A.cur, ref);
    const uint4 r5 = rv[5];
    const uint32_t C = rv[7].y, length = r5.w;
    Surface X1;
    uint32_t matref;
    if (C == 0u || length < 2u || !surf_load(sc, A.surf, dom, X1, matref)) return false;
    job_init(s, x0_of(sc, x, y), X1, matref, ref, length, rv[0].y, dom, r5.x & 0xffu, false);
    return true;
}
__device__ __forceinline__ bool job_hyb(const Job &s) { return s.k >= 2u && s.k < s.length; }
__device__ __forceinline__ bool rough_under(const Surface &X, uint32_t lobe) {
    return (lobe == LOBE_LAMBERT ? 1.0f : X.mat.rough) >= RECONNECTION_ROUGHNESS;
}
__device__ __forceinline__ bool safe_edge(bool ra, bool rb, f3 a, f3 b) {
    return length(a - b) >= RECONNECTION_DISTANCE && ra && rb;
}
__device__ __forceinline__ float rc_geo(f3 prev, const Surface &Xk) {
    const f3 dv = Xk.pos - prev;
    const float d2 = dot(dv, dv);
    const float ck = fabsf(dot(Xk.nrm, dv / __builtin_sqrtf(d2)));
    return d2 / ck;
}
__device__ __forceinline__ uint4 rc_next(const uint4 *rv, uint32_t w20) {
    return (w20 & kResReuseLayout) ? rv[0] : rv[6];
}

enum : int { JK_ANY = -1, JK_L = 0, JK_C = 1, JK_B = 2 };
__device__ __forceinline__ int job_kind(uint32_t length, uint32_t k) {
    return length <= 2u ? JK_L : (k == 2u ? JK_C : JK_B);
}
template <int KIND = JK_ANY>
__device__ __forceinline__ bool job_emit(const Scene &sc, const Seg &g, const ReuseArgs &A, bool emit, Job &s,
                                         uint32_t jid, uint32_t seed0) {
    bool ray = false, vis = false, go = false;
    f3 o = mk(0.0f, 0.0f, 0.0f), d = o, Le = o;
    float remain = -1.0f;
    if (emit) {
        const uint4 *rv = res_of(A, s.ref);
        const f3 V = normalize(s.prev - s.cur.pos);
        const bool hyb = job_hyb(s);
        bool ok = true;
        if (KIND == JK_ANY ? s.i + 1u < s.length : KIND != JK_L) {
            const bool conn = KIND == JK_ANY ? s.shift && hyb && s.i + 1u == s.k : KIND == JK_C;
            const bool fixd = KIND == JK_ANY && s.shift && hyb && s.i == s.k;
            f3 dir;
            uint32_t lobe = LOBE_LAMBERT;
            if (conn || fixd) {
                const uint4 r5 = rv[5];
                const Surface Xt = get_surface(sc, gdecode(conn ? rv[4] : rc_next(rv, r5.x)));
                if (conn) {
                    const bool rk1 = rough_under(s.cur, r5.y), rk = rough_under(Xt, r5.z);
                    if (s.i >= 2u && s.lab == 0u && safe_edge(s.rok, rk1, s.prev, s.cur.pos)) s.lab = s.i;
                    if (s.lab == 0u && safe_edge(rk1, rk, s.cur.pos, Xt.pos)) s.lab = s.k;
                    ok = s.lab == s.k;
                }
                const f3 dv = Xt.pos - s.cur.pos;
                dir = dv / length(dv);
            } else {
                uint32_t seed = s.i == 1u ? seed0 : s.seed1;
                dir = sample_bsdf(seed, s.cur, V, lobe);
            }
            float pdf;
            const f3 fv = bsdf_pdf(s.cur, V, dir, pdf);
            if (!conn && !fixd && (!hyb || s.i + 2u <= s.k)) s.prod *= pdf;
            ok = rr_step(s, s.cur, dir, fv, pdf) && ok;
            if (s.shift && !conn && !fixd) {
                const bool rl = rough_under(s.cur, lobe);
                if (s.i >= 2u && s.lab == 0u && safe_edge(s.rok, rl, s.prev, s.cur.pos)) s.lab = s.i;
                s.rok = rl;
            }
            s.phase = conn ? 2u : (fixd ? 3u : 0u);
            o = s.cur.pos; d = dir;
            ray = ok && !fixd;
            go = ok;
        } else {
            const LightSample XL = load_xl(rv);
            if (s.shift && !hyb) {
                const uint32_t ll = XL.type == LIGHT_ENV ? (s.k == s.length ? rv[5].y : LOBE_GGX) : LOBE_LAMBERT;
                const bool rl = rough_under(s.cur, ll);
                if (s.i >= 2u && s.lab == 0u && safe_edge(s.rok, rl, s.prev, s.cur.pos)) s.lab = s.i;
                if (s.lab == 0u) {
                    const bool rough = s.cur.mat.rough >= RECONNECTION_ROUGHNESS;
                    const bool dirl = XL.type == LIGHT_DIRECTION || XL.type == LIGHT_ENV;
                    if ((dirl || length(s.cur.pos - XL.pos) >= RECONNECTION_DISTANCE) && rough) s.lab = s.length;
                }
                ok = s.lab == s.k;
            }
            const f3 L = direction_to_light(s.cur, XL);
            if (XL.type == LIGHT_ENV) {
                float pdf;
                const f3 fv = bsdf_pdf(s.cur, V, L, pdf);
                ok = rr_step(s, s.cur, L, fv, pdf) && ok;
            }
            s.f = s.f * (bsdf(s.cur, L, V) * fabsf(dot(s.cur.nrm, L)));
            float gl = 1.0f;
            if (XL.type == LIGHT_RECT) {
                const f3 r = XL.pos - s.cur.pos;
                const f3 Ld = normalize(r);
                gl = fabsf(dot(get_light(sc, (uint32_t)XL.id).dir, Ld)) / dot(r, r);
            }
            s.prod = hyb ? s.prod / s.beta : s.prod / (gl * s.beta);
            Le = l_emit<true>(XL, s.cur);
            s.phase = 1u;
            const float dist = length(XL.pos - s.cur.pos);
            o = s.cur.pos; d = (XL.pos - s.cur.pos) / dist; remain = dist;
            vis = true;
            ray = go = ok;
        }
        if (!go) A.jres[jid] = make_float4(0.0f, 0.0f, 0.0f, 0.0f);
    }
    const uint32_t idx = g.rbase + wave_alloc(g.l_ray, ray ? 1u : 0u);
    if (ray) {
        s.idx = idx;
        put_ray(g.rays, idx, o, d, remain, vis ? Q_VIS : Q_CLOSEST);
        if (vis) g.res_out[2u * idx] = make_float4(0.0f, Le.x, Le.y, Le.z);
    }
    return go;
}

__device__ __forceinline__ void job_finish(const Seg &g, const JobLists &JL, const ReuseArgs &A, bool live,
                                           const Job &s, uint32_t jid) {
    if (live) job_store(A, jid, s);
    const bool fold = live && A.fold_last && s.phase == 1u;
    if (fold) A.jres[jid] = make_float4(asf(s.idx), asf(g.out_sel), 0.0f, asf(kJobPending));
    job_keep(g, JL, live && !fold, live && s.phase == 1u, jid);
}

#ifndef JOB_STEP_WAVES
#define JOB_STEP_WAVES 4
#endif
template <bool LDS_SHADE>
__device__ __forceinline__ uint32_t job_step_segment(const Scene &gsc, const WaveBufs &w, uint32_t round,
                                                     const ReuseArgs &A, uint32_t *lds, uint32_t *shade_lds) {
    const JobLists JL = job_lists(w, lds);
    const Scene sc = shading_scene<LDS_SHADE>(gsc, shade_lds, seg_n_in(w, round) != 0u);
    const Seg g = seg_begin(w, round, lds);
    uint32_t nh;
    const uint32_t n = split_count(g, nh);
    for (uint32_t base = 0; base < n; base += WB) {
        const uint32_t q = base + threadIdx.x;
        bool emit = false;
        uint32_t jid = 0u;
        Job s;
        if (q < n) {
            jid = split_at(g, JL, q, nh);
            job_load(sc, A, jid, s);
            if (s.phase != 1u) {
                bool ok = true;
                Surface next;
                uint32_t nref = 0u;
                if (s.phase == 0u) {
                    const Hit h = get_hit(g.res_in, s.idx);
                    ok = h.valid;
                    if (ok) {
                        next = surface_at(sc, h.s, h.pos);
                        nref = mat_index(sc, h.s.inst, h.s.mat);
                    }
                } else {
                    const uint4 *rv = res_of(A, s.ref);
                    const Compact cc = gdecode(s.phase == 2u ? rv[4] : rc_next(rv, rv[5].x));
                    next = get_surface(sc, cc);
                    nref = mat_index(sc, cc.inst, cc.mat);
                    if (s.phase == 2u) {
                        const Hit h = get_hit(g.res_in, s.idx);
                        ok = !(h.valid && h.t < length(next.pos - s.cur.pos) * 0.999f);
                    }
                }
                if (!ok) {
                    A.jres[jid] = make_float4(0.0f, 0.0f, 0.0f, 0.0f);
                } else {
                    const f3 V = normalize(s.prev - s.cur.pos);
                    const f3 L = normalize(next.pos - s.cur.pos);
                    s.f = s.f * (bsdf(s.cur, L, V) * fabsf(dot(s.cur.nrm, L)));
                    if (s.phase == 2u || (!s.shift && job_hyb(s) && s.i + 1u == s.k))
                        s.prod = s.prod * rc_geo(s.cur.pos, next);
                    s.prev = s.cur.pos;
                    s.cur = next;
                    s.matref = nref;
                    s.i += 1u;
                    emit = true;
                }
            } else {
                const float4 a = g.res_in[2u * s.idx];
                s.f = s.f * (mk(a.y, a.z, a.w) * a.x);
                const float qv = s.prod;
                const bool valid = qv > 0.0f && qv <= 3.402823466e38f;
                A.jres[jid] = valid ? make_float4(s.f.x, s.f.y, s.f.z, qv) : make_float4(0.0f, 0.0f, 0.0f, 0.0f);
            }
        }
        const bool live = job_emit(sc, g, A, emit, s, jid, 0u);
        job_finish(g, JL, A, live, s, jid);
    }
    job_seg_end(w, g, JL);
    return *g.l_ray;
}
template <bool LDS_SHADE>
__global__ __launch_bounds__(WB) __attribute__((amdgpu_waves_per_eu(JOB_STEP_WAVES, 8)))
void wjob_step(Scene sc, WaveBufs w, uint32_t round, ReuseArgs A) {
    PTX_WAVE_TIMER(sc, KID_JOB_STEP | (w.seg_base ? 0x80u : 0u));
    __shared__ uint32_t lds[3];
    extern __shared__ __attribute__((aligned(16))) uint32_t shade_lds[];
    (void)job_step_segment<LDS_SHADE>(sc, w, round, A, lds, shade_lds);
}

__device__ __forceinline__ uint32_t reuse_seed(const Scene &sc, uint32_t x, uint32_t y, uint32_t salt) {
    return pcg(pcg(x * 1973u + y * 9277u + sc.U[U_FRAME] * 26699u) ^ salt);
}
__device__ __forceinline__ bool wrs_update(float &w_sum, float wt, uint32_t &seed) {
    w_sum += wt;
    return rnd(seed) < wt / w_sum;
}
struct SelF { bool known; f3 f; };
__device__ __forceinline__ SelF job_f(float4 r) { return SelF{r.w > 0.0f, mk(r.x, r.y, r.z)}; }
__device__ __forceinline__ float4 job_result(const ReuseArgs &A, const WaveBufs &w, float4 r, uint32_t jid) {
    if (asu(r.w) != kJobPending || asu(r.x) >= A.ray_cap || asu(r.y) >= w.nres) return r;
    const float4 a = w.res[asu(r.y)][2u * asu(r.x)], fv = A.jstate[JS_F * (size_t)A.njobs + jid];
    const f3 f = mk(fv.x, fv.y, fv.z) * (mk(a.y, a.z, a.w) * a.x);
    const float qv = fv.w;
    const bool valid = qv > 0.0f && qv <= 3.402823466e38f;
    return valid ? make_float4(f.x, f.y, f.z, qv) : make_float4(0.0f, 0.0f, 0.0f, 0.0f);
}
__device__ __forceinline__ float4 job_at(const ReuseArgs &A, const WaveBufs &w, uint32_t pix, uint32_t slot) {
    const uint32_t jid = job_id(A, pix, slot);
    return job_result(A, w, A.jres[jid], jid);
}
__device__ __forceinline__ SelF stored_f(const uint4 *r) {
    const uint4 r6 = r[6], r7 = r[7];
    return SelF{r7.w == 1u, mk(asf(r6.z), asf(r6.w), asf(r7.z))};
}
__device__ __forceinline__ uint32_t write_reused(uint4 *out, const uint4 *src, float p_sel, float q_sel, SelF fs,
                                                 float w_sum, uint32_t C) {
    uint4 a0 = src[0], a5 = src[5];
    const uint4 a1 = src[1], a2 = src[2], a3 = src[3], a4 = src[4];
    if (fs.known && !(a5.x & kResReuseLayout)) {
        const uint32_t k = a5.x & 0xffu;
        if (k >= 2u && k + 1u < a5.w) a0 = src[6];
        a5.x |= kResReuseLayout;
    }
    out[0] = a0; out[1] = a1; out[2] = a2; out[3] = a3; out[4] = a4; out[5] = a5;
    out[6] = make_uint4(asu(p_sel), asu(q_sel), fs.known ? asu(fs.f.x) : 0u, fs.known ? asu(fs.f.y) : 0u);
    out[7] = make_uint4(asu(p_sel > 0.0f ? w_sum / p_sel : 0.0f), C, fs.known ? asu(fs.f.z) : 0u, fs.known ? 1u : 0u);
    return a5.w;
}

constexpr uint32_t kNbrEscape = 0xFFFFFFFFu;
__device__ __forceinline__ uint4 nbr_pack(bool valid, uint4 r5, uint4 r6, uint4 r7) {
    uint32_t w = 0u;
    const uint32_t k = r5.x & 0xffu;
    if (valid)
        w = (r5.w > 0xfu || k > 0xfu || r7.y > 0x7ffffeu) ? kNbrEscape : (1u << 31) | (r5.w << 27) | (k << 23) | r7.y;
    return make_uint4(r6.x, r6.y, r7.x, w);
}

__device__ __forceinline__ bool temporal_from_init(const Scene &sc, const WaveBufs &w, const ReuseArgs &A, Job &s,
                                                   uint32_t pix, uint32_t jid) {
    const uint4 *rv = res_at(A.cur, s.ref);
    const bool hyb = job_hyb(s);
    while (s.i + 1u < s.length) {
        f3 V = normalize(s.prev - s.cur.pos);
        uint32_t seed = s.i == 1u ? rv[0].x : s.seed1, lobe;
        const f3 dir = sample_bsdf(seed, s.cur, V, lobe);
        float pdf;
        const f3 fv = bsdf_pdf(s.cur, V, dir, pdf);
        if (!hyb || s.i + 2u <= s.k) s.prod *= pdf;
        if (!rr_step(s, s.cur, dir, fv, pdf)) {
            A.jres[jid] = make_float4(0.0f, 0.0f, 0.0f, 0.0f);
            return false;
        }
        const float4 c = w.state[(s.i == 1u ? kStateCs2 : kStateCs3) * w.npix + pix];
        const Surface next = get_surface(sc, gdecode(make_uint4(asu(c.x), asu(c.y), asu(c.z), asu(c.w))));
        V = normalize(s.prev - s.cur.pos);
        const f3 L = normalize(next.pos - s.cur.pos);
        s.f = s.f * (bsdf(s.cur, L, V) * fabsf(dot(s.cur.nrm, L)));
        if (hyb && s.i + 1u == s.k) s.prod = s.prod * rc_geo(s.cur.pos, next);
        s.prev = s.cur.pos;
        s.cur = next;
        s.i += 1u;
    }
    const float T = w.state[kStateTsel * w.npix + pix].x;
    if (T < 0.0f) return true;
    const LightSample XL = load_xl(rv);
    const f3 V = normalize(s.prev - s.cur.pos);
    const f3 L = direction_to_light(s.cur, XL);
    s.f = s.f * (bsdf(s.cur, L, V) * fabsf(dot(s.cur.nrm, L)));
    float gl = 1.0f;
    if (XL.type == LIGHT_RECT) {
        const f3 r = XL.pos - s.cur.pos;
        const f3 Ld = normalize(r);
        gl = fabsf(dot(get_light(sc, (uint32_t)XL.id).dir, Ld)) / dot(r, r);
    }
    s.prod = hyb ? s.prod / s.beta : s.prod / (gl * s.beta);
    const f3 Le = l_emit<true>(XL, s.cur);
    s.f = s.f * (Le * T);
    const float qv = s.prod;
    const bool valid = qv > 0.0f && qv <= 3.402823466e38f;
    A.jres[jid] = valid ? make_float4(s.f.x, s.f.y, s.f.z, qv) : make_float4(0.0f, 0.0f, 0.0f, 0.0f);
    return false;
}

template <bool LDS_SHADE>
__global__ __launch_bounds__(WB) __attribute__((amdgpu_waves_per_eu(2, 8)))
void wtemporal_start(Scene gsc, WaveBufs w, ReuseArgs A) {
    PTX_WAVE_TIMER(gsc, KID_TEMP_START | (w.seg_base ? 0x80u : 0u));
    __shared__ uint32_t lds[3];
    extern __shared__ __attribute__((aligned(16))) uint32_t shade_lds[];
    const JobLists JL = job_lists(w, lds);
    const Scene sc = shading_scene<LDS_SHADE>(gsc, shade_lds, true);
    const Seg g = seg_begin(w, 0u, lds);
    const uint32_t np = padded_pixels(sc);
    for (uint32_t k = 0; k < w.seg_px; k += WB) {
        const uint32_t q = seg_pixel(w, g.j, k);
        uint32_t x, y, pix = 0u;
        bool active = false;
        Job s;
        if (q < np && tile_xy(sc, q, x, y)) {
            pix = (y - sc.row_begin) * sc.width + x;
            active = job_begin(sc, A, s, x, y, (int32_t)pix, (int32_t)pix);
            if (active && A.use_init) active = temporal_from_init(sc, w, A, s, pix, pix);
        }
        const bool live = job_emit(sc, g, A, active, s, pix, active ? A.cur[8u * (size_t)pix].x : 0u);
        job_finish(g, JL, A, live, s, pix);
    }
    job_seg_end(w, g, JL);
}

__global__ __launch_bounds__(WB) void wtemporal_combine(Scene sc, WaveBufs w, ReuseArgs A) {
    PTX_WAVE_TIMER(sc, KID_TEMP_COMBINE | (w.seg_base ? 0x80u : 0u));
    const uint32_t j = w.seg_base + blockIdx.x, np = padded_pixels(sc);
    for (uint32_t k = 0; k < w.seg_px; k += WB) {
        const uint32_t q = seg_pixel(w, j, k);
        uint32_t x, y;
        if (q >= np || !tile_xy(sc, q, x, y)) continue;
        const uint32_t pix = (y - sc.row_begin) * sc.width + x;
        if (!gdecode(A.gbuf[pix]).valid) {
            A.nbr_out[pix] = make_uint4(0u, 0u, 0u, 0u);
            continue;
        }
        uint4 *rv = A.cur + 8u * (size_t)pix;
        const uint4 *hv = A.hist + 8u * (size_t)pix;
        uint32_t seed = reuse_seed(sc, x, y, SALT_TEMPORAL);
        const uint4 r5 = rv[5], r7 = rv[7];
        const float4 er = (r7.y != 0u && r5.w >= 2u) ? job_result(A, w, A.jres[pix], pix) : make_float4(0.0f, 0.0f, 0.0f, 0.0f);
        const float2 ec = make_float2(er.w > 0.0f ? luminance(mk(er.x, er.y, er.z)) : 0.0f, er.w);
        const bool canon_ok = ec.y > 0.0f && ec.x > 0.0f;
        const uint4 h5 = hv[5], h6 = hv[6], h7 = hv[7];
        const uint32_t Cp = A.hist_valid ? min(h7.y, A.cap) : 0u;
        const float cp = (float)Cp, tot = 1.0f + cp;
        const float pp = asf(h6.x), qp = asf(h6.y);
        const bool hist_ok = Cp != 0u && h5.w >= 2u && pp > 0.0f;
        const float wc = canon_ok ? (1.0f / tot) * ec.x * asf(r7.x) : 0.0f;
        const float wp = hist_ok ? (cp / tot) * pp * asf(h7.x) : 0.0f;
        float w_sum = 0.0f, p_sel = ec.x, q_sel = ec.y;
        bool from_hist = false;
        if (wrs_update(w_sum, wc, seed)) { from_hist = false; p_sel = ec.x; q_sel = ec.y; }
        if (wrs_update(w_sum, wp, seed)) { from_hist = true; p_sel = pp; q_sel = qp; }
        write_reused(rv, from_hist ? hv : rv, p_sel, q_sel, from_hist ? stored_f(hv) : job_f(er), w_sum, 1u + Cp);
        const float W = p_sel > 0.0f ? w_sum / p_sel : 0.0f;
        A.nbr_out[pix] = nbr_pack(true, make_uint4(from_hist ? h5.x : r5.x, 0u, 0u, from_hist ? h5.w : r5.w),
                                  make_uint4(asu(p_sel), asu(q_sel), 0u, 0u), make_uint4(asu(W), 1u + Cp, 0u, 0u));
    }
}

__device__ __forceinline__ f3 x0_prev(const ReuseArgs &A, const Scene &sc, uint32_t x, uint32_t y) {
    float u = ((float)x + 0.5f) / (float)sc.U[U_W];
    float v = ((float)y + 0.5f) / (float)sc.U[U_H];
    return xform_point(A.vpinv_prev, mk(2.0f * u - 1.0f, 2.0f * v - 1.0f, 0.0f));
}
struct MotionHist { bool ok; int32_t pp; uint32_t px, py, C; };
__device__ __forceinline__ MotionHist motion_hist(const Scene &sc, const ReuseArgs &A, const Surface &X1, uint32_t y,
                                                  bool count = false) {
    MotionHist m{false, 0, 0u, 0u, 0u};
    if (!A.hist_valid) return m;
    const float *vp = A.vp_prev;
    const f3 P = X1.pos;
    const float cx = ((vp[0] * P.x + vp[4] * P.y) + vp[8] * P.z) + vp[12];
    const float cy = ((vp[1] * P.x + vp[5] * P.y) + vp[9] * P.z) + vp[13];
    const float cw = ((vp[3] * P.x + vp[7] * P.y) + vp[11] * P.z) + vp[15];
    if (!(cw > 0.0f)) return m;
    const float W = (float)sc.width, H = (float)sc.height;
    const float fx = ((cx / cw + 1.0f) * 0.5f) * W, fy = ((cy / cw + 1.0f) * 0.5f) * H;
    if (!(fx >= 0.0f && fx < W && fy >= 0.0f && fy < H)) return m;
    m.px = (uint32_t)fx;
    m.py = (uint32_t)fy;
    const int32_t ry = (int32_t)m.py - (int32_t)sc.row_begin;
    if (abs((int32_t)m.py - (int32_t)y) > (int32_t)A.radius || ry < A.prev_row_lo || ry >= A.prev_row_hi) {
        if (count && A.clip) atomicAdd(A.clip, 1ull);
        return m;
    }
    m.pp = ry * (int32_t)sc.width + (int32_t)m.px;
    const uint4 a = A.psurf[2 * (ptrdiff_t)m.pp];
    if (a.w == kNoSurface) return m;
    const uint4 b = A.psurf[2 * (ptrdiff_t)m.pp + 1];
    const f3 pp = mk(asf(a.x), asf(a.y), asf(a.z)), pn = mk(asf(b.x), asf(b.y), asf(b.z));
    if (!(dot(pn, X1.nrm) >= 0.9f)) return m;
    const f3 x0p = x0_prev(A, sc, m.px, m.py);
    const float dp = length(pp - x0p), dc = length(P - x0p);
    if (!(fabsf(dp - dc) <= 0.05f * dc)) return m;
    m.C = min(A.hist[8 * (ptrdiff_t)m.pp + 7].y, A.cap);
    m.ok = m.C != 0u;
    return m;
}

#ifndef MOTION_START_WAVES
#define MOTION_START_WAVES 3
#endif
template <bool LDS_SHADE>
__global__ __launch_bounds__(WB) __attribute__((amdgpu_waves_per_eu(MOTION_START_WAVES, 8)))
void wtmotion_start(Scene gsc, WaveBufs w, ReuseArgs A) {
    PTX_WAVE_TIMER(gsc, KID_TEMP_START | (w.seg_base ? 0x80u : 0u));
    __shared__ uint32_t lds[3];
    extern __shared__ __attribute__((aligned(16))) uint32_t shade_lds[];
    const JobLists JL = job_lists(w, lds);
    const Scene sc = shading_scene<LDS_SHADE>(gsc, shade_lds, true);
    const Seg g = seg_begin(w, 0u, lds);
    const uint32_t np = padded_pixels(sc);
    for (uint32_t k = 0; k < w.seg_px; k += WB) {
        const uint32_t q = seg_pixel(w, g.j, k);
        uint32_t x = 0u, y = 0u, pix = 0u;
        bool valid = false;
        Surface X1{};
        uint32_t mref = 0u;
        if (q < np && tile_xy(sc, q, x, y)) {
            pix = (y - sc.row_begin) * sc.width + x;
            valid = surf_load(sc, A.surf, pix, X1, mref);
        }
        const uint4 *rv = A.cur + 8u * (size_t)pix;
        const uint4 r5c = valid ? rv[5] : make_uint4(0u, 0u, 0u, 0u);
        const uint32_t cC = valid ? rv[7].y : 0u, clen = r5c.w, ck = r5c.x & 0xffu;
        const bool canon = valid && cC != 0u && clen >= 2u;
        const MotionHist mh = valid ? motion_hist(sc, A, X1, y, true) : MotionHist{false, 0, 0u, 0u, 0u};
#pragma unroll 1
        for (uint32_t slot = 0; slot < kMotionJobs; ++slot) {
            const uint32_t jid = job_id(A, pix, slot);
            Job s;
            bool act = false;
            uint32_t s0 = 0u;
            if (slot == 0u) {
                act = canon && job_begin(sc, A, s, x, y, (int32_t)pix, (int32_t)pix);
                if (act && A.use_init) act = temporal_from_init(sc, w, A, s, pix, jid);
                if (act) s0 = rv[0].x;
            } else if (slot == 1u) {
                if (mh.ok) {
                    const uint4 *hv = A.hist + 8 * (ptrdiff_t)mh.pp;
                    const uint4 h0 = hv[0], h5 = hv[5], h6 = hv[6];
                    act = h5.w >= 2u && asf(h6.x) > 0.0f;
                    if (act) {
                        job_init(s, x0_of(sc, x, y), X1, mref, kHistRef + mh.pp, h5.w, h0.y, (int32_t)pix, h5.x & 0xffu,
                                 true);
                        s0 = h0.x;
                    }
                }
            } else if (mh.ok && canon) {
                Surface Xp;
                uint32_t pref;
                act = surf_load(sc, A.psurf, mh.pp, Xp, pref);
                if (act) {
                    job_init(s, x0_prev(A, sc, mh.px, mh.py), Xp, pref, (int32_t)pix, clen, rv[0].y, kDomPrev, ck, true);
                    s0 = rv[0].x;
                }
            }
            const bool live = job_emit(sc, g, A, act, s, jid, s0);
            job_finish(g, JL, A, live, s, jid);
        }
    }
    job_seg_end(w, g, JL);
}

__global__ __launch_bounds__(WB) void wtmotion_combine(Scene sc, WaveBufs w, ReuseArgs A) {
    PTX_WAVE_TIMER(sc, KID_TEMP_COMBINE | (w.seg_base ? 0x80u : 0u));
    const uint32_t j = w.seg_base + blockIdx.x, np = padded_pixels(sc);
    for (uint32_t k = 0; k < w.seg_px; k += WB) {
        const uint32_t q = seg_pixel(w, j, k);
        uint32_t x, y;
        if (q >= np || !tile_xy(sc, q, x, y)) continue;
        const uint32_t pix = (y - sc.row_begin) * sc.width + x;
        Surface X1;
        uint32_t mref;
        if (!surf_load(sc, A.surf, pix, X1, mref)) {
            A.nbr_out[pix] = make_uint4(0u, 0u, 0u, 0u);
            continue;
        }
        uint4 *rv = A.cur + 8u * (size_t)pix;
        uint32_t seed = reuse_seed(sc, x, y, SALT_TEMPORAL);
        const uint4 r5 = rv[5], r7 = rv[7];
        const float4 er = (r7.y != 0u && r5.w >= 2u) ? job_at(A, w, pix, 0u) : make_float4(0.0f, 0.0f, 0.0f, 0.0f);
        const float ecp = er.w > 0.0f ? luminance(mk(er.x, er.y, er.z)) : 0.0f, ecq = er.w;
        const bool canon_ok = ecq > 0.0f && ecp > 0.0f;
        const float cc = 1.0f, pc = ecp, qc = ecq, Wc = asf(r7.x);
        const MotionHist mh = motion_hist(sc, A, X1, y);
        const uint32_t Cp = mh.ok ? mh.C : 0u;
        const float cp = (float)Cp;
        const uint4 *hv = A.hist + 8 * (ptrdiff_t)mh.pp;
        float wh = 0.0f, pf = 0.0f, qf = 0.0f;
        SelF ff{false, mk(0.0f, 0.0f, 0.0f)};
        uint32_t hlen = 0u, hk = 0u;
// ... 543 lines not shown
```

pathtracerdemo_amd/csrc/ptx_stream.h:

```cpp
#pragma once
#include "ptx_wave_common.h"

namespace ptx {

#ifndef PTX_STREAM_REFILL
#define PTX_STREAM_REFILL 32
#endif
#ifndef PTX_TRACE_STREAM
#define PTX_TRACE_STREAM 1
#endif
template <bool PROF, bool OCC>
__device__ __forceinline__ void trace_stream(const Scene &sc, const SubRoot *subs, const Inst *insts, PassEps eps,
                                             uint32_t *stack, CoopLds coop, const WaveBufs &w, float4 *res_all,
                                             uint32_t *l_next, uint32_t sj, uint32_t sn) {
    const uint32_t lane = __lane_id();
    bool src_done = false;
    uint32_t qbase = 0u, qleft = 0u;
    bool has = false;
    uint32_t gi = 0u, kind = 0u, seg = 0u;
    float T = 1.0f, remain = 0.0f;
    Ray ray{mk(0.0f, 0.0f, 0.0f), mk(0.0f, 0.0f, 1.0f)};
    Prof pf{};
    FlatWalk wk;
    for (;;) {
        const unsigned long long walking = wballot(has && !wk.done);
        const uint32_t waiting = (uint32_t)__popcll(wballot(!(has && !wk.done)));
        if (walking == 0ull || (waiting >= PTX_STREAM_REFILL && !src_done)) {
            if (has && wk.done) {
                if (PROF) wk.count(sc);
                if (end_query(sc, subs, insts, eps, wk.hit(), ray, kind, T, remain, seg, res_all, gi)) has = false;
                else wk.begin(ray, vis_bound(remain));
            }
            unsigned long long want = wballot(!has);
            while (want != 0ull && !src_done) {
                if (qleft == 0u) {
                    uint32_t b = 0u;
                    if (lane == 0u) b = __hip_atomic_fetch_add(l_next, 1u, __ATOMIC_RELAXED, __HIP_MEMORY_SCOPE_WORKGROUP);
                    b = (uint32_t)__builtin_amdgcn_readfirstlane((int)b);
                    if (b * 64u >= sn) {
                        src_done = true;
                        break;
                    }
                    qbase = sj * w.ray_stride + b * 64u;
                    qleft = min(64u, sn - b * 64u);
                }
                const uint32_t m = (uint32_t)__popcll(want), take = min(m, qleft);
                const uint32_t rank = __builtin_amdgcn_mbcnt_hi((uint32_t)(want >> 32), __builtin_amdgcn_mbcnt_lo((uint32_t)want, 0u));
                if (!has && rank < take) {
                    gi = qbase + rank;
                    const float4 a = w.rays[2u * gi], b = w.rays[2u * gi + 1u];
                    ray = Ray{mk(a.x, a.y, a.z), mk(b.x, b.y, b.z)};
                    remain = a.w;
                    kind = asu(b.w);
                    T = 1.0f;
                    seg = 0u;
                    has = true;
                    wk.begin(ray, kind != Q_CLOSEST ? vis_bound(remain) : 1e10f);
                }
                qbase += take;
                qleft -= take;
                want = wballot(!has);
            }
            if (wballot(has) == 0ull) break;
        }
        wk.refill<PROF>(sc, subs, insts, ray, pf);
        wk.nodes<PROF>(sc, subs, stack, WB, pf);
        wk.leaves<PROF, OCC>(sc, coop, eps, remain, pf);
    }
    if (PROF) prof_flush(sc, pf);
}

}
```

pathtracerdemo_amd/csrc/ptx_wave.hip:

```cpp
#include "ptx_stream.h"

#include <algorithm>
#include <cstdlib>

namespace ptx {

#ifndef TRACE_OCC_WAVES
#define TRACE_OCC_WAVES 5
#endif
template <bool COUNT, bool PROF, bool OCC, bool LDS_TABLES>
__device__ __forceinline__ void trace_lanes(const Scene &sc, const SubRoot *subs, const Inst *insts, PassEps eps,
                                            uint32_t *stack, CoopLds coop, Ray r, uint32_t kind, float T, float remain,
                                            uint32_t seg, bool active, float4 *res, uint32_t gi) {
    for (;;) {
        const float t_max = !active ? __builtin_nanf("") : kind != Q_CLOSEST ? vis_bound(remain) : 1e10f;
        const Hit h = (LDS_TABLES && !COUNT)
                          ? trace_core_flat<PROF, OCC>(sc, subs, insts, r, eps, stack, WB, t_max, coop, remain)
                          : trace_core_tab<COUNT, PROF, true, OCC, true>(sc, subs, insts, r, eps, stack, WB, t_max, coop,
                                                                         false, remain);
        if (active && end_query(sc, subs, insts, eps, h, r, kind, T, remain, seg, res, gi)) active = false;
        if (wballot(active) == 0ull) break;
    }
}
template <bool COUNT, bool PROF, bool OCC, bool LDS_TABLES>
__device__ __forceinline__ void trace_batch(const Scene &sc, const SubRoot *subs, const Inst *insts, PassEps eps,
                                            uint32_t *stack, CoopLds coop, float4 *res_all, const float4 *rays_all,
                                            uint32_t gbase, uint32_t i, bool active) {
    const uint32_t gi = gbase + i;
    float4 a = make_float4(0.0f, 0.0f, 0.0f, 0.0f), b = make_float4(0.0f, 0.0f, 1.0f, 0.0f);
    if (active) {
        a = rays_all[2u * gi];
        b = rays_all[2u * gi + 1u];
    }
    trace_lanes<COUNT, PROF, OCC, LDS_TABLES>(sc, subs, insts, eps, stack, coop, Ray{mk(a.x, a.y, a.z), mk(b.x, b.y, b.z)},
                                              asu(b.w), 1.0f, a.w, 0u, active, res_all, gi);
}

template <bool COUNT, int WAVES, bool PROF = false, bool LDS_TABLES = true, bool OCC = false>
__global__ __launch_bounds__(WB) __attribute__((amdgpu_waves_per_eu(WAVES, 8)))
void trace_queue(Scene sc, WaveBufs w, uint32_t round, PassEps eps) {
    PTX_WAVE_TIMER(sc, KID_TRACE | (w.seg_base ? 0x80u : 0u));
    extern __shared__ __attribute__((aligned(16))) uint32_t wstack[];
    const uint32_t tw = LDS_TABLES ? tables_lds_bytes(sc) / 4u : 0u;
    uint32_t *stack = wstack + tw + threadIdx.x;
    __shared__ unsigned long long c_key[WB];
    __shared__ uint32_t c_mark[WB];
    const CoopLds coop{c_key + (threadIdx.x & ~63u), c_mark + (threadIdx.x & ~63u)};
    const uint32_t j = w.seg_phys + w.seg_base + blockIdx.x;
    const uint32_t n = w.cnt[(2u * round + 1u) * w.cnt_stride + j];
    if (n == 0u) return;
    __shared__ uint32_t l_next;
    if (threadIdx.x == 0u) l_next = 0u;
    const LdsTables T = LDS_TABLES ? stage_tables(sc, wstack) : LdsTables{sc.subs, sc.insts};
    const SubRoot *subs = T.subs;
    const Inst *insts = T.insts;
    if constexpr (PTX_TRACE_STREAM && LDS_TABLES && !COUNT) {
        trace_stream<PROF, OCC>(sc, subs, insts, eps, stack, coop, w, res_buf(w, round), &l_next, j, n);
        return;
    }
    if (COUNT && sc.census)
        sc.counters = sc.census + (size_t)kCensusWords * ((sc.row_end - sc.row_begin + 7u) / 8u + j);
    for (uint32_t i0 = 0u; i0 < n; i0 += WB) {
        const uint32_t i = i0 + threadIdx.x;
        trace_batch<COUNT, PROF, OCC, LDS_TABLES>(sc, subs, insts, eps, stack, coop, res_buf(w, round), w.rays,
                                                   j * w.ray_stride, i, i < n);
    }
}

template <bool COUNT>
__global__ __launch_bounds__(WB) void trace_queue_sm(Scene sc, const float4 *rays_all, float4 *res_all,
                                                     uint32_t stride, uint32_t n_total, PassEps eps) {
    extern __shared__ __attribute__((aligned(16))) uint32_t wstack[];
    uint32_t *stack = wstack + threadIdx.x;
    const uint32_t j = blockIdx.x;
    const uint32_t n = min(stride, n_total - j * stride);
    const float4 *rays = rays_all + 2u * (size_t)j * stride;
    float4 *res = res_all + 2u * (size_t)j * stride;
    const float vx = 1e-4f;
    const uint32_t n_inst = sc.n_inst;

    uint32_t next = threadIdx.x, cur = 0u;
    bool have = false;
    Ray r{};
    uint32_t ii = 0u, s = 0u, nsub = 0u, grp = 0u, sub_base = 0u, tri_base = 0u;
    f3 lo{}, ld{}, inv{};
    int sp = -1;
    uint32_t tcount = 0u, tprim = 0u, tidx = 0u;
    float vy = 1e10f;
    bool bvalid = false;
    uint32_t binst = 0u, bmat = 0u, bprim = 0u;
    uint32_t n_aabb = 0u, n_tri = 0u;

    for (;;) {
        if (!have && next < n) {
            cur = next;
            next += WB;
            const float4 a = rays[2u * cur], b = rays[2u * cur + 1u];
            r = Ray{mk(a.x, a.y, a.z), mk(a.w, b.x, b.y)};
            have = true;
            ii = 0xffffffffu; s = 0u; nsub = 0u; sp = -1; tcount = 0u;
            vy = 1e10f;
            bvalid = false; n_aabb = 0u; n_tri = 0u;
        }
        if (__ballot(have) == 0ull) break;
        if (!have) continue;

        bool do_node = false;
        uint32_t node = 0u;
        if (tcount == 0u) {
            if (sp >= 0) {
                const uint32_t ref = stack[(uint32_t)sp * WB];
                --sp;
                if (ref & LEAF_BIT) {
                    tcount = (ref >> 24) & 0x7Fu;
                    tprim = ref & LEAF_FIRST_MASK;
                    tidx = 3u * (tri_base + tprim);
                } else {
                    do_node = true;
                    node = ref;
                }
            } else if (s < nsub) {
                const SubRoot &R = sc.subs[sub_base + s];
                grp = s;
                ++s;
                ++n_aabb;
                if (box_root(lo, inv, R, vx, vy)) {
                    sp = 0;
                    stack[0] = R.ref;
                }
            } else if (ii + 1u < n_inst) {
                ii = ii + 1u;
                const Inst &I = sc.insts[ii];
                lo = xform_point(I.minv, r.o);
                const f3 le = xform_point(I.minv, r.o + r.d);
                ld = le - lo;
                inv = mk(1.0f / ld.x, 1.0f / ld.y, 1.0f / ld.z);
                nsub = I.nsub;
                sub_base = I.sub_base;
                tri_base = I.tri_base;
                s = 0u;
            } else {
                if (COUNT) {
                    atomicAdd(&sc.counters[CNT_RAYS], 1ull);
                    atomicAdd(&sc.counters[CNT_INST], (unsigned long long)n_inst);
                    atomicAdd(&sc.counters[CNT_AABB], (unsigned long long)n_aabb);
                    atomicAdd(&sc.counters[CNT_TRI], (unsigned long long)n_tri);
                    if (bvalid) atomicAdd(&sc.counters[CNT_HITS], 1ull);
                }
                Hit h;
                h.valid = bvalid;
                h.t = bvalid ? vy : 0.0f;
                h.s = Compact{0u, bvalid ? binst : 0u, bvalid ? bmat : 0u, bvalid ? bprim : 0u, 0.0f, 0.0f};
                h.pos = mk(0.0f, 0.0f, 0.0f);
                if (bvalid) complete_hit(sc, r, eps, h);
                const uint32_t enc = ((h.valid ? 1u : 0u) << 31) | (h.s.inst << 16) | h.s.mat;
                res[2u * cur] = make_float4(h.t, asf(enc), asf(h.s.prim), h.s.bu);
                res[2u * cur + 1u] = make_float4(h.s.bv, h.pos.x, h.pos.y, h.pos.z);
                have = false;
                continue;
            }
        }
        if (tcount > 0u) {
            const float4 a = sc.tris[tidx], b = sc.tris[tidx + 1u], c = sc.tris[tidx + 2u];
            const float t = ray_tri(lo, ld, a, b, c, eps.det_eps);
            ++n_tri;
            if (!(vy < t)) {
                vy = t;
                bvalid = true;
                binst = ii;
                bmat = grp;
                bprim = tprim;
            }
            tidx += 3u;
            ++tprim;
            --tcount;
        } else if (do_node) {
            const float4 *np = reinterpret_cast<const float4 *>(sc.nodes + node);
            const float4 q0 = np[0], q1 = np[1], q2 = np[2], q3 = np[3];
            const uint32_t lref = __float_as_uint(q3.x), rref = __float_as_uint(q3.y);
            float tl, tr;
            bool hl, hr;
            box_pair(lo, inv, q0, q1, q2, vx, vy, hl, hr, tl, tr);
            n_aabb += 2u;
            if (hl && hr) {
                stack[(uint32_t)(sp + 1) * WB] = tl < tr ? rref : lref;
                stack[(uint32_t)(sp + 2) * WB] = tl < tr ? lref : rref;
                sp += 2;
            } else if (hl || hr) {
                stack[(uint32_t)(sp + 1) * WB] = hl ? lref : rref;
                sp += 1;
            }
        }
    }
}

template <bool ROOTQ>
__global__ __launch_bounds__(WB) void wgbuffer(Scene sc, WaveBufs w, uint4 *gbuf) {
    PTX_WAVE_TIMER(sc, KID_GBUF);
    extern __shared__ __attribute__((aligned(16))) uint32_t wstack[];
    uint32_t *stack = wstack + tables_lds_bytes(sc) / 4u + threadIdx.x;
    const LdsTables T = stage_tables(sc, wstack);
    const uint32_t L = blockIdx.x * 4u + threadIdx.x / 64u, run = w.cluster * w.seg_count;
    const uint32_t t = set_tile(w, (L / run) * w.cluster * w.nseg + w.cluster * w.seg_base + L % run);
    const uint32_t q = t * 64u + (threadIdx.x & 63u);
    uint32_t x, y;
    if (q >= padded_pixels(sc) || !tile_xy(sc, q, x, y)) return;
    const float *vpinv = reinterpret_cast<const float *>(sc.U + U_VPINV);
    const float u = ((float)x + 0.5f) / (float)sc.U[U_W];
    const float v = ((float)y + 0.5f) / (float)sc.U[U_H];
    const f3 st = xform_point(vpinv, mk(2.0f * u - 1.0f, 2.0f * v - 1.0f, 0.0f));
    const f3 en = xform_point(vpinv, mk(2.0f * u - 1.0f, 2.0f * v - 1.0f, 0.0f + 1.0f));
    const Hit h = trace_core_tab<false, false, ROOTQ>(sc, T.subs, T.insts, Ray{st, normalize(en - st)},
                                                      PassEps{1e-8f, 1e-6f}, stack, WB);
    Compact c = h.s;
    c.valid = h.valid ? 1u : 0u;
    gbuf[(y - sc.row_begin) * sc.width + x] = gencode(c);
}

// ... 299 lines not shown
        uint32_t seed = s.i == 1u ? resv[0].x : s.seed1;
        uint32_t lobe;
        const f3 dir = sample_bsdf(seed, s.cur, V, lobe);
        s.phase = 0u;
        put_ray(rays, idx, s.cur.pos, dir, -1.0f, Q_CLOSEST);
    } else {
        const LightSample XL = load_xl(resv);
        const f3 L = direction_to_light(s.cur, XL);
        s.f = s.f * (bsdf(s.cur, L, V) * fabsf(dot(s.cur.nrm, L)));
        const f3 Le = l_emit<true>(XL, s.cur);
        s.phase = 1u;
        const float dist = length(XL.pos - s.cur.pos);
        put_ray(rays, idx, s.cur.pos, (XL.pos - s.cur.pos) / dist, dist, Q_VIS);
        res[2u * idx] = make_float4(0.0f, Le.x, Le.y, Le.z);
    }
}
__device__ __forceinline__ void wfinal_store(float4 *state, uint32_t npix, uint32_t pix, const WFinal &s,
                                             uint32_t matref) {
    state[FS_HDR * npix + pix] = make_float4(asf(s.i | (s.length << 8) | (s.phase << 16)), asf(s.seed1),
                                             asf(s.idx), 0.0f);
    state[FS_F * npix + pix] = make_float4(s.f.x, s.f.y, s.f.z, s.ucw);
    if (s.phase != 0u) return;
    state[FS_CUR * npix + pix] = make_float4(s.cur.pos.x, s.cur.pos.y, s.cur.pos.z, asf(matref));
    state[FS_NRM * npix + pix] = make_float4(s.cur.nrm.x, s.cur.nrm.y, s.cur.nrm.z, 0.0f);
    state[FS_PREV * npix + pix] = make_float4(s.prev.x, s.prev.y, s.prev.z, 0.0f);
}

__global__ __launch_bounds__(WB) __attribute__((amdgpu_waves_per_eu(LOGIC_WAVES, 8))) void wfinal_start(Scene sc, WaveBufs w, const uint4 *gbuf, const uint4 *reservoir,
                                                   float4 *accum) {
    PTX_WAVE_TIMER(sc, KID_FINAL_START | (w.seg_base ? 0x80u : 0u));
    __shared__ uint32_t lds[3];
    const JobLists JL = job_lists(w, lds);
    const Seg g = seg_begin(w, 0u, lds);
    float4 *state = w.state;
    const uint32_t npix = w.npix, np = padded_pixels(sc);
    for (uint32_t k = 0; k < w.seg_px; k += WB) {
        const uint32_t q = seg_pixel(w, g.j, k);
        uint32_t x, y, pix = 0u, matref = 0u;
        bool active = false;
        WFinal s;
        if (q < np && tile_xy(sc, q, x, y)) {
            pix = (y - sc.row_begin) * sc.width + x;
            const Compact x1 = gdecode(gbuf[pix]);
            const uint4 *rv = reservoir + 8u * (size_t)pix;
            if (!x1.valid) {
                accum[pix] = make_float4(ENV_C, ENV_C, ENV_C, 1.0f);
            } else {
                const uint4 r0 = rv[0], r5 = rv[5], r7 = rv[7];
                s.length = r5.w;
                if (r7.y == 0u || s.length < 2u) {
                    mix_color(sc, accum, pix, mk(0.0f, 0.0f, 0.0f));
                } else if (r7.w == 1u) {
                    const uint4 r6 = rv[6];
                    mix_color(sc, accum, pix, mk(asf(r6.z), asf(r6.w), asf(r7.z)) * asf(r7.x));
                } else {
                    active = true;
                    s.seed1 = r0.y;
                    s.ucw = asf(r7.x);
                    s.prev = x0_of(sc, x, y);
                    s.cur = get_surface(sc, x1);
                    matref = mat_index(sc, x1.inst, x1.mat);
                    s.f = mk(1.0f, 1.0f, 1.0f);
                    s.i = 1u;
                }
            }
        }
        wfinal_emit(sc, g, active, s, reservoir + 8u * (size_t)pix);
        if (active) wfinal_store(state, npix, pix, s, matref);
        job_keep(g, JL, active, active && s.phase != 0u, pix);
    }
    job_seg_end(w, g, JL);
}

__global__ __launch_bounds__(WB) __attribute__((amdgpu_waves_per_eu(LOGIC_WAVES, 8))) void wfinal_step(Scene sc, WaveBufs w, uint32_t round, const uint4 *reservoir,
                                                  float4 *accum) {
    PTX_WAVE_TIMER(sc, KID_FINAL_STEP | (w.seg_base ? 0x80u : 0u));
    __shared__ uint32_t lds[3];
    const JobLists JL = job_lists(w, lds);
    const Seg g = seg_begin(w, round, lds);
    float4 *state = w.state;
    const float4 *res_in = g.res_in;
    const uint32_t npix = w.npix;
    uint32_t nh;
    const uint32_t n = split_count(g, nh);
    for (uint32_t base = 0; base < n; base += WB) {
        const uint32_t q = base + threadIdx.x;
        bool emit = false;
        uint32_t pix = 0u, matref = 0u;
        WFinal s;
        if (q < n) {
            pix = split_at(g, JL, q, nh);
            const float4 hd = state[FS_HDR * npix + pix], fv = state[FS_F * npix + pix];
            const uint32_t hw = asu(hd.x);
            s.i = hw & 0xffu; s.length = (hw >> 8) & 0xffu; s.phase = hw >> 16;
            s.seed1 = asu(hd.y); s.idx = asu(hd.z);
            s.f = mk(fv.x, fv.y, fv.z); s.ucw = fv.w;
            if (s.phase == 0u) {
                const float4 cu = state[FS_CUR * npix + pix], nr = state[FS_NRM * npix + pix];
                const float4 pv = state[FS_PREV * npix + pix];
                s.prev = mk(pv.x, pv.y, pv.z);
                matref = asu(cu.w);
                s.cur.pos = mk(cu.x, cu.y, cu.z);
                s.cur.nrm = mk(nr.x, nr.y, nr.z);
                s.cur.mat = material_at(sc, matref);
            }
            if (s.phase == 0u) {
                const Hit h = get_hit(res_in, s.idx);
                const Surface next = h.valid ? surface_at(sc, h.s, h.pos) : get_surface(sc, h.s);
                const f3 V = normalize(s.prev - s.cur.pos);
                const f3 L = normalize(next.pos - s.cur.pos);
                s.f = s.f * (bsdf(s.cur, L, V) * fabsf(dot(s.cur.nrm, L)));
                s.prev = s.cur.pos;
                s.cur = next;
                matref = mat_index(sc, h.s.inst, h.s.mat);
                s.i += 1u;
                emit = true;
            } else {
                const float4 a = res_in[2u * s.idx];
                s.f = s.f * (mk(a.y, a.z, a.w) * a.x);
                mix_color(sc, accum, pix, s.f * s.ucw);
            }
        }
        wfinal_emit(sc, g, emit, s, reservoir + 8u * (size_t)pix);
        if (emit) wfinal_store(state, npix, pix, s, matref);
        job_keep(g, JL, emit, emit && s.phase != 0u, pix);
    }
    job_seg_end(w, g, JL);
}

__device__ __forceinline__ void wfinal_walk(const Scene &sc, const LdsTables &T, const PassEps &eps, uint32_t *stack,
                                            const CoopLds &coop, float4 *rays, float4 *res, uint32_t slot,
                                            const uint4 *resv, float4 *accum, uint32_t pix, bool active, WFinal &s) {
    for (uint32_t it = 0u; it < (uint32_t)kWaveRoundsFinal; ++it) {
        if (wballot(active) == 0ull) break;
        if (active) {
            const f3 V = normalize(s.prev - s.cur.pos);
            if (s.i + 1u < s.length) {
                uint32_t seed = s.i == 1u ? resv[0].x : s.seed1;
                uint32_t lobe;
                const f3 dir = sample_bsdf(seed, s.cur, V, lobe);
                s.phase = 0u;
                put_ray(rays, slot, s.cur.pos, dir, -1.0f, Q_CLOSEST);
            } else {
                const LightSample XL = load_xl(resv);
                const f3 L = direction_to_light(s.cur, XL);
                s.f = s.f * (bsdf(s.cur, L, V) * fabsf(dot(s.cur.nrm, L)));
                const f3 Le = l_emit<true>(XL, s.cur);
                s.phase = 1u;
                const float dist = length(XL.pos - s.cur.pos);
                put_ray(rays, slot, s.cur.pos, (XL.pos - s.cur.pos) / dist, dist, Q_VIS);
                res[2u * slot] = make_float4(0.0f, Le.x, Le.y, Le.z);
            }
        }
        trace_batch<false, false, false, true>(sc, T.subs, T.insts, eps, stack, coop, res, rays, 0u, slot, active);
        if (active) {
            if (s.phase == 0u) {
                const Hit h = get_hit(res, slot);
                const Surface next = h.valid ? surface_at(sc, h.s, h.pos) : get_surface(sc, h.s);
                const f3 V = normalize(s.prev - s.cur.pos);
                const f3 L = normalize(next.pos - s.cur.pos);
                s.f = s.f * (bsdf(s.cur, L, V) * fabsf(dot(s.cur.nrm, L)));
                s.prev = s.cur.pos;
                s.cur = next;
                s.i += 1u;
            } else {
                const float4 a = res[2u * slot];
                s.f = s.f * (mk(a.y, a.z, a.w) * a.x);
                mix_color(sc, accum, pix, s.f * s.ucw);
                active = false;
            }
        }
    }
}

__global__ __launch_bounds__(WB) __attribute__((amdgpu_waves_per_eu(2, 8)))
void wfinal_one(Scene sc, WaveBufs w, const uint4 *gbuf, const uint4 *reservoir, float4 *accum, PassEps eps) {
    PTX_WAVE_TIMER(sc, KID_FINAL_START | (w.seg_base ? 0x80u : 0u));
    extern __shared__ __attribute__((aligned(16))) uint32_t wstack[];
    __shared__ unsigned long long c_key[WB];
    __shared__ uint32_t c_mark[WB];
    const LdsTables T = stage_tables(sc, wstack);
    uint32_t *stack = wstack + tables_lds_bytes(sc) / 4u + threadIdx.x;
    const CoopLds coop{c_key + (threadIdx.x & ~63u), c_mark + (threadIdx.x & ~63u)};
    const uint32_t j = w.seg_base + blockIdx.x, pj = w.seg_phys + j, np = padded_pixels(sc);
    float4 *rays = w.rays + 2u * (size_t)pj * w.ray_stride, *res = w.res[0] + 2u * (size_t)pj * w.ray_stride;
    const uint32_t slot = threadIdx.x;
    for (uint32_t k = 0; k < w.seg_px; k += WB) {
        const uint32_t q = seg_pixel(w, j, k);
        uint32_t x, y, pix = 0u;
        bool active = false;
        WFinal s;
        if (q < np && tile_xy(sc, q, x, y)) {
            pix = (y - sc.row_begin) * sc.width + x;
            const Compact x1 = gdecode(gbuf[pix]);
            const uint4 *rv = reservoir + 8u * (size_t)pix;
            if (!x1.valid) {
                accum[pix] = make_float4(ENV_C, ENV_C, ENV_C, 1.0f);
            } else {
                const uint4 r0 = rv[0], r5 = rv[5], r7 = rv[7];
                s.length = r5.w;
                if (r7.y == 0u || s.length < 2u) {
                    mix_color(sc, accum, pix, mk(0.0f, 0.0f, 0.0f));
                } else if (r7.w == 1u) {
                    const uint4 r6 = rv[6];
                    mix_color(sc, accum, pix, mk(asf(r6.z), asf(r6.w), asf(r7.z)) * asf(r7.x));
                } else {
                    active = true;
                    s.seed1 = r0.y;
                    s.ucw = asf(r7.x);
                    s.prev = x0_of(sc, x, y);
                    s.cur = get_surface(sc, x1);
                    s.f = mk(1.0f, 1.0f, 1.0f);
                    s.i = 1u;
                }
            }
        }
        wfinal_walk(sc, T, eps, stack, coop, rays, res, slot, reservoir + 8u * (size_t)pix, accum, pix, active, s);
    }
}

__global__ __launch_bounds__(WB) __attribute__((amdgpu_waves_per_eu(2, 8)))
void wfinal_replay(Scene sc, WaveBufs w, const uint4 *gbuf, const uint4 *reservoir, float4 *accum,
                   const uint32_t *replay, uint32_t *replay_cnt, PassEps eps) {
    PTX_WAVE_TIMER(sc, KID_FINAL_START | (w.seg_base ? 0x80u : 0u));
    extern __shared__ __attribute__((aligned(16))) uint32_t wstack[];
    __shared__ unsigned long long c_key[WB];
    __shared__ uint32_t c_mark[WB];
    const uint32_t pj = w.seg_phys + w.seg_base + blockIdx.x;
    const uint32_t n = min(replay_cnt[pj], w.seg_px);
    if (n == 0u) return;
    const LdsTables T = stage_tables(sc, wstack);
    __syncthreads();
    if (threadIdx.x == 0u) replay_cnt[pj] = 0u;
    uint32_t *stack = wstack + tables_lds_bytes(sc) / 4u + threadIdx.x;
    const CoopLds coop{c_key + (threadIdx.x & ~63u), c_mark + (threadIdx.x & ~63u)};
    float4 *rays = w.rays + 2u * (size_t)pj * w.ray_stride, *res = w.res[0] + 2u * (size_t)pj * w.ray_stride;
    const uint32_t slot = threadIdx.x;
    const uint32_t *list = replay + (size_t)pj * w.seg_px;
    for (uint32_t k = 0; k < n; k += WB) {
        const uint32_t e = k + threadIdx.x < n ? list[k + threadIdx.x] : w.npix;
        const bool active = e < w.npix;
        const uint32_t pix = active ? e : 0u;
        WFinal s;
        if (active) {
            const uint4 *rv = reservoir + 8u * (size_t)pix;
            s.length = rv[5].w;
            s.seed1 = rv[0].y;
            s.ucw = asf(rv[7].x);
            s.prev = x0_of(sc, pix % sc.width, sc.row_begin + pix / sc.width);
            s.cur = get_surface(sc, gdecode(gbuf[pix]));
            s.f = mk(1.0f, 1.0f, 1.0f);
            s.i = 1u;
        }
        wfinal_walk(sc, T, eps, stack, coop, rays, res, slot, reservoir + 8u * (size_t)pix, accum, pix, active, s);
    }
}

enum : uint32_t { MS_HDR, MS_COL, MS_FP, MS_ORG, MS_COUNT };
struct WMcpt {
    uint32_t seed, bounce, flags, lbase, pidx;
    f3 color, f;
    float p;
    f3 org;
};
__device__ __forceinline__ void wmcpt_store(float4 *state, uint32_t npix, uint32_t pix, const WMcpt &s) {
    state[MS_HDR * npix + pix] = make_float4(asf(s.seed), asf(s.bounce | (s.flags << 8)), asf(s.lbase), asf(s.pidx));
    state[MS_COL * npix + pix] = make_float4(s.color.x, s.color.y, s.color.z, 0.0f);
    state[MS_FP * npix + pix] = make_float4(s.f.x, s.f.y, s.f.z, s.p);
    state[MS_ORG * npix + pix] = make_float4(s.org.x, s.org.y, s.org.z, 0.0f);
}
__device__ __forceinline__ void mcpt_light_ray(const Scene &sc, uint32_t &seed, const Surface &X, f3 V, f3 fp,
                                               uint32_t id, uint32_t idx, float4 *rays, float4 *res) {
    const Light ls = get_light(sc, id);
    LightSample XL;
    XL.type = ls.type;
    XL.Le = ls.color * ls.intensity;
    XL.pos = mk(0.0f, 0.0f, 0.0f);
    XL.dir = mk(0.0f, 0.0f, 0.0f);
    XL.pdf = 0.0f;
    if (ls.type == LIGHT_DIRECTION) {
        XL.pos = X.pos - ls.dir * INF_F; XL.dir = ls.dir; XL.pdf = 1.0f;
    } else if (ls.type == LIGHT_POINT) {
        XL.pos = ls.pos; XL.dir = normalize(X.pos - ls.pos); XL.pdf = 1.0f;
    } else if (ls.type == LIGHT_RECT) {
        const float ru = rnd(seed) * 2.0f - 1.0f;
        const float rv = rnd(seed) * 2.0f - 1.0f;
        XL.pos = ls.pos + (ls.U * ru + ls.V * rv);
        XL.dir = normalize(X.pos - XL.pos);
        const f3 rr = XL.pos - X.pos;
        const f3 Ld = normalize(rr);
        XL.pdf = dot(rr, rr) / fmaxf(ls.area * fabsf(dot(ls.dir, Ld)), EPS_F);
    }
    const f3 L = direction_to_light(X, XL);
    f3 c = l_emit<false>(XL, X) * bsdf(X, V, L);
    c = c * fabsf(dot(X.nrm, L));
    const float dist = length(XL.pos - X.pos);
    put_ray(rays, idx, X.pos, (XL.pos - X.pos) / dist, dist, Q_VIS);
    res[2u * idx] = make_float4(0.0f, c.x, c.y, c.z);
    res[2u * idx + 1u] = make_float4(XL.pdf, fp.x, fp.y, fp.z);
}

__device__ __forceinline__ void wmcpt_vertex(const Scene &sc, const Seg &g, bool emit, WMcpt &s, const Surface &X) {
    float4 *rays = g.rays, *res = g.res_out;
    const uint32_t nl = sc.U[U_LIGHT_COUNT];
    const uint32_t lbase = g.rbase + wave_alloc(g.l_ray, emit ? nl : 0u);
    bool path_ray = false;
    f3 Lb = mk(0.0f, 0.0f, 0.0f);
// ... 249 lines not shown
```

pathtracerdemo_amd/csrc/ptx_wave_common.h:

```cpp
#pragma once
#include "ptx_launch.h"
#include "ptx_shading.h"

namespace ptx {

constexpr uint32_t WB = kBlock;
#ifndef LOGIC_WAVES
#define LOGIC_WAVES 4
#endif
enum : uint32_t { Q_CLOSEST = 0u, Q_VIS = 1u, Q_OCC = 2u };

__device__ __forceinline__ uint32_t wave_scan(uint32_t v, uint32_t &total) { return wave_excl_sum(v, total); }
__device__ __forceinline__ uint32_t wave_alloc(uint32_t *lds_ctr, uint32_t n) {
    uint32_t total;
    const uint32_t excl = wave_scan(n, total);
    uint32_t base = 0u;
    if (__lane_id() == 0u && total) base = atomicAdd(lds_ctr, total);
    base = (uint32_t)__builtin_amdgcn_readfirstlane((int)base);
    return base + excl;
}

struct Seg {
    uint32_t j, round;
    uint32_t pj;
    uint32_t rbase;
    float4 *rays, *res_out;
    const float4 *res_in;
    uint32_t out_sel;
    uint32_t *act_out;
    const uint32_t *act_in;
    uint32_t n_in;
    uint32_t *l_ray, *l_act;
};
__device__ __forceinline__ uint32_t res_sel(const WaveBufs &w, uint32_t round) {
    return w.nres == 3u ? round % 3u : round & 1u;
}
__device__ __forceinline__ float4 *res_buf(const WaveBufs &w, uint32_t round) { return w.res[res_sel(w, round)]; }
__device__ __forceinline__ uint32_t seg_n_in(const WaveBufs &w, uint32_t round) {
    return round ? w.cnt[(2u * (round - 1u)) * w.cnt_stride + w.seg_phys + w.seg_base + blockIdx.x] : 0u;
}
__device__ __forceinline__ Seg seg_begin(const WaveBufs &w, uint32_t round, uint32_t *lds) {
    Seg g;
    g.j = w.seg_base + blockIdx.x;
    g.pj = w.seg_phys + g.j;
    g.round = round;
    g.rbase = g.pj * w.ray_stride;
    g.rays = w.rays;
    g.res_out = res_buf(w, round);
    g.res_in = round ? res_buf(w, round - 1u) : w.res[1];
    g.out_sel = res_sel(w, round);
    g.act_out = w.act[round & 1u] + (size_t)g.pj * w.act_stride;
    g.act_in = w.act[(round + 1u) & 1u] + (size_t)g.pj * w.act_stride;
    g.n_in = seg_n_in(w, round);
    g.l_ray = lds;
    g.l_act = lds + 1;
    if (threadIdx.x == 0) { lds[0] = 0u; lds[1] = 0u; }
    __syncthreads();
    return g;
}
__device__ __forceinline__ void seg_end(const WaveBufs &w, const Seg &g) {
    __syncthreads();
    if (threadIdx.x == 0) {
        w.cnt[(2u * g.round) * w.cnt_stride + g.pj] = *g.l_act;
        w.cnt[(2u * g.round + 1u) * w.cnt_stride + g.pj] = *g.l_ray;
    }
}
__device__ __forceinline__ uint32_t set_tile(const WaveBufs &w, uint32_t v) {
    return v < w.ntile0 ? w.tile0 + v : v - w.ntile0 < w.ntile1 ? w.tile1 + (v - w.ntile0) : 0x3ffffffu;
}
__device__ __forceinline__ uint32_t seg_pixel(const WaveBufs &w, uint32_t j, uint32_t k) {
    const uint32_t s = (k + threadIdx.x) >> 6;
    const uint32_t cl = w.cluster;
    const uint32_t t = set_tile(w, ((s / cl) * w.nseg + j) * cl + s % cl);
    return t * 64u + (threadIdx.x & 63u);
}
__device__ __forceinline__ void seg_keep(const Seg &g, bool keep, uint32_t pix) {
    const uint32_t slot = wave_alloc(g.l_act, keep ? 1u : 0u);
    if (keep) g.act_out[slot] = pix;
}

struct JobLists { uint32_t *l_light; uint32_t stride; };
__device__ __forceinline__ JobLists job_lists(const WaveBufs &w, uint32_t *lds) {
    if (threadIdx.x == 0) lds[2] = 0u;
    return JobLists{lds + 2, w.act_stride};
}
__device__ __forceinline__ void job_keep(const Seg &g, const JobLists &L, bool keep, bool light, uint32_t jid) {
    const uint32_t sh = wave_alloc(g.l_act, keep && !light ? 1u : 0u);
    const uint32_t sl = wave_alloc(L.l_light, keep && light ? 1u : 0u);
    if (keep) g.act_out[light ? L.stride - 1u - sl : sh] = jid;
}
__device__ __forceinline__ void job_seg_end(const WaveBufs &w, const Seg &g, const JobLists &L) {
    __syncthreads();
    if (threadIdx.x == 0) {
        w.cnt[(2u * g.round) * w.cnt_stride + g.pj] = *g.l_act | (*L.l_light << 16);
        w.cnt[(2u * g.round + 1u) * w.cnt_stride + g.pj] = *g.l_ray;
    }
}

__device__ __forceinline__ uint32_t split_count(const Seg &g, uint32_t &nh) {
    nh = g.n_in & 0xffffu;
    return nh + (g.n_in >> 16);
}
__device__ __forceinline__ uint32_t split_at(const Seg &g, const JobLists &L, uint32_t q, uint32_t nh) {
    return g.act_in[q < nh ? q : L.stride - 1u - (q - nh)];
}

__device__ __forceinline__ void put_ray(float4 *rays, uint32_t idx, f3 o, f3 d, float remain, uint32_t kind) {
    rays[2u * idx] = make_float4(o.x, o.y, o.z, remain);
    rays[2u * idx + 1u] = make_float4(d.x, d.y, d.z, asf(kind));
}
__device__ __forceinline__ Hit get_hit(const float4 *res, uint32_t idx) {
    const float4 a = res[2u * idx], b = res[2u * idx + 1u];
    const uint32_t enc = asu(a.y);
    Hit h;
    h.valid = (enc >> 31) != 0u;
    h.t = a.x;
    h.s = Compact{enc >> 31, (enc >> 16) & 0x7fffu, enc & 0xffffu, asu(a.z), a.w, b.x};
    h.pos = mk(b.y, b.z, b.w);
    return h;
}
#ifndef PTX_LDS_TRANS
#define PTX_LDS_TRANS 1
#endif
__device__ __forceinline__ bool end_query(const Scene &sc, const SubRoot *subs, const Inst *insts, PassEps eps, Hit h,
                                          Ray &ray, uint32_t kind, float &T, float &remain, uint32_t &seg, float4 *res,
                                          uint32_t gi) {
    if (kind == Q_CLOSEST) {
        if (h.valid) complete_hit(sc, ray, eps, h, insts);
        const uint32_t enc = ((h.valid ? 1u : 0u) << 31) | (h.s.inst << 16) | h.s.mat;
        res[2u * gi] = make_float4(h.t, asf(enc), asf(h.s.prim), h.s.bu);
        res[2u * gi + 1u] = make_float4(h.s.bv, h.pos.x, h.pos.y, h.pos.z);
        return true;
    }
    float out = -1.0f;
    if (!h.valid || h.t > remain) out = T;
    else {
        const float tr = kind == Q_OCC    ? 0.0f
                         : PTX_LDS_TRANS ? subs_transmission(subs, insts, h.s.inst, h.s.mat)
                                         : get_transmission(sc, h.s.inst, h.s.mat);
        if (tr == 0.0f) out = 0.0f;
        else {
            T *= tr;
            remain -= h.t;
            complete_hit(sc, ray, eps, h, insts);
            ray.o = h.pos;
            if (seg == 4u) out = 0.0f;
            ++seg;
        }
    }
    if (out < 0.0f) return false;
    res[2u * gi].x = out;
    return true;
}
__device__ __forceinline__ f3 x0_of(const Scene &sc, uint32_t x, uint32_t y) {
    const float *vpinv = reinterpret_cast<const float *>(sc.U + U_VPINV);
    float u = ((float)x + 0.5f) / (float)sc.U[U_W];
    float v = ((float)y + 0.5f) / (float)sc.U[U_H];
    return xform_point(vpinv, mk(2.0f * u - 1.0f, 2.0f * v - 1.0f, 0.0f));
}
__device__ __forceinline__ Compact gdecode(uint4 g) {
    return Compact{(g.x & 0x80000000u) ? 1u : 0u, (g.x & 0x7fff0000u) >> 16, g.x & 0xffffu, g.y, asf(g.z), asf(g.w)};
}
__device__ __forceinline__ uint4 gencode(const Compact &s) {
    return make_uint4((s.valid << 31) | (s.inst << 16) | s.mat, s.prim, asu(s.bu), asu(s.bv));
}
__device__ __forceinline__ float mix_weight(const Scene &sc) { return 1.0f / (float)(sc.U[U_FRAME] + 1u); }
__device__ __forceinline__ float4 mixed_color(float4 a, f3 c, float t) {
    return make_float4(mixf(a.x, c.x, t), mixf(a.y, c.y, t), mixf(a.z, c.z, t), 1.0f);
}
__device__ __forceinline__ void mix_color(const Scene &sc, float4 *accum, uint32_t i, f3 c) {
    accum[i] = mixed_color(accum[i], c, mix_weight(sc));
    if (sc.frame_color) sc.frame_color[i] = make_float4(c.x, c.y, c.z, 1.0f);
}
__device__ __forceinline__ bool tile_xy(const Scene &sc, uint32_t p, uint32_t &x, uint32_t &y) {
    const uint32_t tiles_x = (sc.width + 7u) / 8u, t = p >> 6, l = p & 63u;
    x = (t % tiles_x) * 8u + (l & 7u);
    y = sc.row_begin + (t / tiles_x) * 8u + (l >> 3);
    return x < sc.width && y < sc.row_end;
}
__device__ __forceinline__ uint32_t padded_pixels(const Scene &sc) {
    return ((sc.width + 7u) / 8u) * ((sc.row_end - sc.row_begin + 7u) / 8u) * 64u;
}

constexpr uint32_t kNoSurface = 0xFFFFFFFFu;
__device__ __forceinline__ void surf_store(uint4 *surf, ptrdiff_t i, const Surface &X, uint32_t matref) {
    surf[2 * i] = make_uint4(asu(X.pos.x), asu(X.pos.y), asu(X.pos.z), matref);
    surf[2 * i + 1] = make_uint4(asu(X.nrm.x), asu(X.nrm.y), asu(X.nrm.z), 0u);
}
__device__ __forceinline__ void surf_store_none(uint4 *surf, ptrdiff_t i) {
    surf[2 * i] = make_uint4(0u, 0u, 0u, kNoSurface);
}
__device__ __forceinline__ bool surf_load(const Scene &sc, const uint4 *surf, ptrdiff_t i, Surface &X,
                                          uint32_t &matref) {
    const uint4 a = surf[2 * i];
    if (a.w == kNoSurface) return false;
    const uint4 b = surf[2 * i + 1];
    X.pos = mk(asf(a.x), asf(a.y), asf(a.z));
    X.nrm = mk(asf(b.x), asf(b.y), asf(b.z));
    X.mat = material_at(sc, a.w);
    matref = a.w;
    return true;
}
__device__ __forceinline__ void surf_from_gbuf(const Scene &sc, uint4 *surf, ptrdiff_t i, uint4 g) {
    const Compact x1 = gdecode(g);
    if (!x1.valid) surf_store_none(surf, i);
    else surf_store(surf, i, get_surface(sc, x1), mat_index(sc, x1.inst, x1.mat));
}

__device__ __forceinline__ LightSample load_xl(const uint4 *res) {
    const uint4 r1 = res[1], r2 = res[2], r3 = res[3];
    LightSample XL;
    XL.dir = mk(asf(r1.x), asf(r1.y), asf(r1.z));
    XL.type = r1.w;
    XL.pos = mk(asf(r2.x), asf(r2.y), asf(r2.z));
    XL.id = (int32_t)r2.w;
    XL.Le = mk(asf(r3.x), asf(r3.y), asf(r3.z));
    XL.pdf = asf(r3.w);
    return XL;
}
}
```

Measured before the change: 585.0 Msamples/s.

## Write folded visibility results straight into per-job visibility plane

```diff
diff --git a/pathtracerdemo_amd/csrc/ptx_api.cpp b/pathtracerdemo_amd/csrc/ptx_api.cpp
--- a/pathtracerdemo_amd/csrc/ptx_api.cpp
+++ b/pathtracerdemo_amd/csrc/ptx_api.cpp
@@ -615,11 +615,12 @@
         for (DevBuf &r : c.wres) free_buf(r);
         c.wave_ray_cap = 0;
         if (int rc = alloc_buf(h, c.wrays, cap * 32u)) return rc;
-        for (int i = 0; i < (h->cfg.pipeline == PTX_PIPELINE_RESTIR_REUSE ? 3 : 2); ++i)
-            if (int rc = alloc_buf(h, c.wres[i], cap * 32u)) return rc;
+        for (DevBuf &r : c.wres)
+            if (int rc = alloc_buf(h, r, cap * 32u)) return rc;
         c.wave_ray_cap = cap;
     }
     w.surf = nullptr;
+    w.jvis = nullptr;
     if (h->cfg.pipeline == PTX_PIPELINE_RESTIR_REUSE) {
         const size_t rows = (size_t)h->halo_top + h->band_h + h->halo_bot;
         if (c.surf.bytes != rows * h->cfg.width * 32u) c.surf_valid = false;
@@ -632,8 +633,7 @@
     w.nseg = (uint32_t)nseg;
     w.ray_stride = (uint32_t)(per_px * seg_px);
     w.rays = (float4 *)c.wrays.p;
-    for (int i = 0; i < 3; ++i) w.res[i] = (float4 *)c.wres[i].p;
-    w.nres = 2;
+    for (int i = 0; i < 2; ++i) w.res[i] = (float4 *)c.wres[i].p;
     for (int i = 0; i < 2; ++i) w.act[i] = (uint32_t *)c.wact[i].p;
     w.act_stride = (uint32_t)(seg_px * jpp);
     w.cnt = (uint32_t *)c.wctr.p;
@@ -676,6 +676,8 @@
     const size_t npix = (size_t)h->band_h * h->cfg.width;
     if (int rc = alloc_buf(h, h->cur().tjstate, npix * kMotionJobs * 6u * 16u)) return rc;
     if (int rc = alloc_buf(h, h->cur().tjres, npix * kMotionJobs * 16u)) return rc;
+    if (int rc = alloc_buf(h, h->cur().tjvis, npix * kMotionJobs * 4u)) return rc;
+    if (int rc = alloc_buf(h, h->d_jvis, njobs * 4u)) return rc;
     return alloc_buf(h, h->d_jres, njobs * 16u);
 }
 static ReuseArgs reuse_args(ptx_handle *h, int pass) {
@@ -686,6 +688,7 @@
     const bool temporal = pass == PTX_PASS_TEMPORAL;
     A.jstate = (float4 *)(temporal ? h->cur().tjstate.p : h->d_jstate.p);
     A.jres = (float4 *)(temporal ? h->cur().tjres.p : h->d_jres.p);
+    A.jvis = (float *)(temporal ? h->cur().tjvis.p : h->d_jvis.p);
     A.jpp = temporal ? 1u : 2u * h->reuse_neighbors;
     A.njobs = h->band_h * h->cfg.width * A.jpp;
     static const bool planes = ab_knob("JOB_PLANES", 1) != 0;
@@ -701,7 +704,6 @@
     A.surf = h->cur().surf.p ? (const uint4 *)h->cur().surf.p + 2u * (size_t)h->halo_top * h->cfg.width : nullptr;
     static const bool fold_off = ab_knob("FOLD_LAST_STEP", 1) == 0;
     A.fold_last = ((pass == PTX_PASS_SPATIAL || pass == PTX_PASS_TEMPORAL) && !fold_off) ? 1u : 0u;
-    A.ray_cap = (uint32_t)std::min<size_t>(h->cur().wave_ray_cap, 0xffffffffu);
     return A;
 }
 
@@ -710,6 +712,7 @@
     ReuseArgs A = reuse_args(h, PTX_PASS_SPATIAL);
     A.jstate = (float4 *)h->cur().tjstate.p;
     A.jres = (float4 *)h->cur().tjres.p;
+    A.jvis = (float *)h->cur().tjvis.p;
     A.jpp = kMotionJobs;
     A.njobs = h->band_h * h->cfg.width * A.jpp;
     static const bool planes = ab_knob("JOB_PLANES", 1) != 0;
@@ -795,7 +798,7 @@
         ReuseArgs A = is_motion_pass(pass) ? motion_args(h)
                                            : reuse_args(h, temporal ? PTX_PASS_TEMPORAL : PTX_PASS_SPATIAL);
         WaveBufs wj = w;
-        if (A.fold_last && wj.res[2]) wj.nres = 3;
+        if (A.fold_last && A.jvis && A.njobs < (1u << 30)) wj.jvis = A.jvis;
         else A.fold_last = 0u;
         if (fused && pass == PTX_PASS_SPATIAL) {
             A.fuse_final = 1u;
@@ -912,7 +915,7 @@
     if (h->cfg.flags & PTX_FLAG_SINGLE_STREAM) k = 1;
     k = std::max(1, std::min<int>({k, ptx_handle::kMaxSplit, (int)interior.nseg, (int)edge.nseg}));
     ReuseArgs A = reuse_args(h, PTX_PASS_SPATIAL);
-    const bool fold = A.fold_last && interior.res[2];
+    const bool fold = A.fold_last && A.jvis && A.njobs < (1u << 30);
     if (!fold) A.fold_last = 0u;
     const int nr = reuse_rounds(0, A);
     if ((e = fork_sequences(h, k)) != hipSuccess) return e;
@@ -926,7 +929,7 @@
         wi.seg_phys = interior.seg_phys + E;
         we.seg_phys = interior.seg_phys + E + wi.seg_base + wi.seg_count - we.seg_base;
         E += we.seg_count;
-        if (fold) wi.nres = we.nres = 3;
+        if (fold) wi.jvis = we.jvis = A.jvis;
         WaveBufs wt = wi;
         wt.seg_count = wi.seg_count + we.seg_count;
         if (surf_stale) {
@@ -2518,7 +2521,7 @@
     const auto &c = h->cur();
     out->device_bytes = h->d_scene.bytes + h->d_geometry.bytes + h->d_tris.bytes + h->d_nodes.bytes + h->d_subs.bytes +
                         h->d_insts.bytes + h->d_mats.bytes + h->d_tverts.bytes + c.gbuf.bytes + c.res.bytes + h->d_accum.bytes +
-                        h->d_hist.bytes + h->d_jstate.bytes + h->d_jres.bytes + c.tjstate.bytes + c.tjres.bytes + c.nbr.bytes +
+                        h->d_hist.bytes + h->d_jstate.bytes + h->d_jres.bytes + h->d_jvis.bytes + c.tjstate.bytes + c.tjres.bytes + c.tjvis.bytes + c.nbr.bytes +
                         c.surf.bytes + h->d_psurf.bytes + c.direct.bytes + h->d_dn_guide.bytes + h->d_dn_work.bytes +
                         h->d_denoised.bytes + h->d_frame_color.bytes + h->d_dn_guide_prev.bytes + h->d_dn_hist[0].bytes +
                         h->d_dn_hist[1].bytes + h->d_dn_mom[0].bytes + h->d_dn_mom[1].bytes + h->d_dn_halo_g.bytes +
@@ -2849,7 +2852,6 @@
     w.ray_stride = kWaveSegPixels;
     w.rays = (float4 *)h->d_qrays.p;
     w.res[0] = w.res[1] = (float4 *)h->d_qhits.p;
-    w.nres = 2;
     w.cnt = (uint32_t *)h->d_qcnt.p;
     TimedLaunch &t = h->ring[h->ring_pos];
     h->ring_pos = (h->ring_pos + 1) % kEventRing;
@@ -2894,15 +2896,15 @@
     if (h->present_host) (void)hipHostFree(h->present_host);
     for (DevBuf *b : {&h->d_canvas, &h->d_canvas_async, &h->d_scene, &h->d_geometry, &h->d_tris, &h->d_nodes, &h->d_subs,
                       &h->d_insts, &h->d_mats, &h->d_tverts, &h->d_accum, &h->d_counters, &h->d_qrays, &h->d_qhits, &h->d_qcnt, &h->d_hist,
-                      &h->d_jstate, &h->d_jres, &h->d_replay, &h->d_psurf, &h->d_census, &h->d_wgt, &h->d_dn_guide, &h->d_dn_work,
+                      &h->d_jstate, &h->d_jres, &h->d_jvis, &h->d_replay, &h->d_psurf, &h->d_census, &h->d_wgt, &h->d_dn_guide, &h->d_dn_work,
                       &h->d_denoised, &h->d_frame_color, &h->d_dn_guide_prev, &h->d_dn_hist[0], &h->d_dn_hist[1], &h->d_dn_mom[0],
                       &h->d_dn_mom[1], &h->d_dn_halo_g, &h->d_dn_halo_c, &h->d_dn_obj, &h->d_dn_snap, &h->d_up_halo, &h->d_ut_guide[0], &h->d_ut_guide[1],
                       &h->d_ut_hist[0], &h->d_ut_hist[1], &h->d_refit_order, &h->d_refit_box})
         free_buf(*b);
     drop_skins(h);
     for (auto &c : h->ctx) {
-        for (DevBuf *b : {&c.gbuf, &c.res, &c.direct, &c.nbr, &c.tjstate, &c.tjres, &c.surf, &c.wstate, &c.wrays, &c.wres[0],
-                          &c.wres[1], &c.wres[2], &c.wact[0], &c.wact[1], &c.wctr})
+        for (DevBuf *b : {&c.gbuf, &c.res, &c.direct, &c.nbr, &c.tjstate, &c.tjres, &c.tjvis, &c.surf, &c.wstate, &c.wrays, &c.wres[0],
+                          &c.wres[1], &c.wact[0], &c.wact[1], &c.wctr})
             free_buf(*b);
         if (c.ev_fork) (void)hipEventDestroy(c.ev_fork);
         for (int q = 0; q < ptx_handle::kMaxSplit; ++q) {
diff --git a/pathtracerdemo_amd/csrc/ptx_internal.h b/pathtracerdemo_amd/csrc/ptx_internal.h
--- a/pathtracerdemo_amd/csrc/ptx_internal.h
+++ b/pathtracerdemo_amd/csrc/ptx_internal.h
@@ -61,7 +61,7 @@
     uint32_t uniform[PTX_UNIFORM_WORDS] = {0};
     bool frame_set = false;
     uint32_t band_h = 0, halo_top = 0, halo_bot = 0;
-    DevBuf d_accum, d_counters, d_hist, d_jstate, d_jres;
+    DevBuf d_accum, d_counters, d_hist, d_jstate, d_jres, d_jvis;
     DevBuf d_replay;
     uint32_t res_u4 = 8;
     bool gbuf_exposed = false;
@@ -82,9 +82,9 @@
     static constexpr int kGbufKeyWords = 32;
     struct FrameCtx {
         DevBuf gbuf, res, direct;
-        DevBuf nbr, tjstate, tjres;
+        DevBuf nbr, tjstate, tjres, tjvis;
         DevBuf surf;
-        DevBuf wstate, wrays, wres[3], wact[2], wctr;
+        DevBuf wstate, wrays, wres[2], wact[2], wctr;
         size_t wave_ray_cap = 0;
         hipStream_t own = nullptr, stream = nullptr;
         hipStream_t sub[kMaxSplit] = {nullptr, nullptr, nullptr, nullptr};
diff --git a/pathtracerdemo_amd/csrc/ptx_launch.h b/pathtracerdemo_amd/csrc/ptx_launch.h
--- a/pathtracerdemo_amd/csrc/ptx_launch.h
+++ b/pathtracerdemo_amd/csrc/ptx_launch.h
@@ -138,14 +138,14 @@
     uint32_t cluster;
     uint32_t ray_stride;
     float4 *rays;
-    float4 *res[3];
-    uint32_t nres;
+    float4 *res[2];
     uint32_t *act[2];
     uint32_t act_stride;
     uint32_t *cnt;
     uint32_t tile0, ntile0, tile1, ntile1;
     uint32_t seg_phys, cnt_stride;
     uint4 *surf;
+    float *jvis;
 };
 hipError_t wave_trace(const Scene &sc, const WaveBufs &w, int round, int eps_mode, uint32_t stack_depth,
                       hipStream_t s, bool occ_only = false);
@@ -171,6 +171,7 @@
     uint4 *hist;
     float4 *jstate;
     float4 *jres;
+    float *jvis;
     uint32_t njobs, jpp;
     uint32_t jpx, jslot;
     uint32_t radius, neighbors, cap, hist_valid;
@@ -179,7 +180,6 @@
     uint4 *nbr_out;
     const uint4 *surf;
     uint32_t fold_last;
-    uint32_t ray_cap;
     uint32_t motion;
     float vpinv_prev[16], vp_prev[16];
     const uint4 *psurf;
@@ -192,7 +192,6 @@
 };
 constexpr uint32_t kMotionJobs = 3u;
 constexpr uint32_t kJobPending = 0xFFFFFFFFu;
-static_assert(kWaveRoundsReuse <= 3, "fold_last: one result buffer per reuse trace round");
 int reuse_rounds(int pass_temporal, const ReuseArgs &A);
 hipError_t wave_reuse_round(const Scene &sc, const WaveBufs &w, int pass_temporal, int round, const ReuseArgs &A,
                             hipStream_t s);
diff --git a/pathtracerdemo_amd/csrc/ptx_reuse.hip b/pathtracerdemo_amd/csrc/ptx_reuse.hip
--- a/pathtracerdemo_amd/csrc/ptx_reuse.hip
+++ b/pathtracerdemo_amd/csrc/ptx_reuse.hip
@@ -237,8 +237,12 @@
     const uint32_t idx = g.rbase + wave_alloc(g.l_ray, ray ? 1u : 0u);
     if (ray) {
         s.idx = idx;
-        put_ray(g.rays, idx, o, d, remain, vis ? Q_VIS : Q_CLOSEST);
-        if (vis) g.res_out[2u * idx] = make_float4(0.0f, Le.x, Le.y, Le.z);
+        const bool fold = vis && A.fold_last;
+        put_ray(g.rays, idx, o, d, remain, (vis ? Q_VIS : Q_CLOSEST) | (fold ? kind_plane_slot(jid) : 0u));
+        if (vis) {
+            float4 *dst = fold ? A.jres + jid : g.res_out + 2u * idx;
+            *dst = fold ? make_float4(Le.x, Le.y, Le.z, asf(kJobPending)) : make_float4(0.0f, Le.x, Le.y, Le.z);
+        }
     }
     return go;
 }
@@ -247,7 +251,6 @@
                                            const Job &s, uint32_t jid) {
     if (live) job_store(A, jid, s);
     const bool fold = live && A.fold_last && s.phase == 1u;
-    if (fold) A.jres[jid] = make_float4(asf(s.idx), asf(g.out_sel), 0.0f, asf(kJobPending));
     job_keep(g, JL, live && !fold, live && s.phase == 1u, jid);
 }
 
@@ -337,17 +340,20 @@
 }
 struct SelF { bool known; f3 f; };
 __device__ __forceinline__ SelF job_f(float4 r) { return SelF{r.w > 0.0f, mk(r.x, r.y, r.z)}; }
-__device__ __forceinline__ float4 job_result(const ReuseArgs &A, const WaveBufs &w, float4 r, uint32_t jid) {
-    if (asu(r.w) != kJobPending || asu(r.x) >= A.ray_cap || asu(r.y) >= w.nres) return r;
-    const float4 a = w.res[asu(r.y)][2u * asu(r.x)], fv = A.jstate[JS_F * (size_t)A.njobs + jid];
-    const f3 f = mk(fv.x, fv.y, fv.z) * (mk(a.y, a.z, a.w) * a.x);
+__device__ __forceinline__ float4 job_result(const ReuseArgs &A, const WaveBufs &w, uint32_t jid) {
+    const float4 r = A.jres[jid];
+    if (!A.fold_last) return r;
+    const float T = w.jvis[jid];
+    const float4 fv = A.jstate[JS_F * (size_t)A.njobs + jid];
+    if (asu(r.w) != kJobPending) return r;
+    const f3 f = mk(fv.x, fv.y, fv.z) * (mk(r.x, r.y, r.z) * T);
     const float qv = fv.w;
     const bool valid = qv > 0.0f && qv <= 3.402823466e38f;
     return valid ? make_float4(f.x, f.y, f.z, qv) : make_float4(0.0f, 0.0f, 0.0f, 0.0f);
 }
 __device__ __forceinline__ float4 job_at(const ReuseArgs &A, const WaveBufs &w, uint32_t pix, uint32_t slot) {
     const uint32_t jid = job_id(A, pix, slot);
-    return job_result(A, w, A.jres[jid], jid);
+    return job_result(A, w, jid);
 }
 __device__ __forceinline__ SelF stored_f(const uint4 *r) {
     const uint4 r6 = r[6], r7 = r[7];
@@ -465,7 +471,7 @@
         const uint4 *hv = A.hist + 8u * (size_t)pix;
         uint32_t seed = reuse_seed(sc, x, y, SALT_TEMPORAL);
         const uint4 r5 = rv[5], r7 = rv[7];
-        const float4 er = (r7.y != 0u && r5.w >= 2u) ? job_result(A, w, A.jres[pix], pix) : make_float4(0.0f, 0.0f, 0.0f, 0.0f);
+        const float4 er = (r7.y != 0u && r5.w >= 2u) ? job_result(A, w, pix) : make_float4(0.0f, 0.0f, 0.0f, 0.0f);
         const float2 ec = make_float2(er.w > 0.0f ? luminance(mk(er.x, er.y, er.z)) : 0.0f, er.w);
         const bool canon_ok = ec.y > 0.0f && ec.x > 0.0f;
         const uint4 h5 = hv[5], h6 = hv[6], h7 = hv[7];
diff --git a/pathtracerdemo_amd/csrc/ptx_stream.h b/pathtracerdemo_amd/csrc/ptx_stream.h
--- a/pathtracerdemo_amd/csrc/ptx_stream.h
+++ b/pathtracerdemo_amd/csrc/ptx_stream.h
@@ -28,7 +28,7 @@
         if (walking == 0ull || (waiting >= PTX_STREAM_REFILL && !src_done)) {
             if (has && wk.done) {
                 if (PROF) wk.count(sc);
-                if (end_query(sc, subs, insts, eps, wk.hit(), ray, kind, T, remain, seg, res_all, gi)) has = false;
+                if (end_query(sc, subs, insts, eps, wk.hit(), ray, kind, T, remain, seg, res_all, gi, w.jvis)) has = false;
                 else wk.begin(ray, vis_bound(remain));
             }
             unsigned long long want = wballot(!has);
@@ -55,7 +55,7 @@
                     T = 1.0f;
                     seg = 0u;
                     has = true;
-                    wk.begin(ray, kind != Q_CLOSEST ? vis_bound(remain) : 1e10f);
+                    wk.begin(ray, (kind & kKindMask) != Q_CLOSEST ? vis_bound(remain) : 1e10f);
                 }
                 qbase += take;
                 qleft -= take;
diff --git a/pathtracerdemo_amd/csrc/ptx_wave.hip b/pathtracerdemo_amd/csrc/ptx_wave.hip
--- a/pathtracerdemo_amd/csrc/ptx_wave.hip
+++ b/pathtracerdemo_amd/csrc/ptx_wave.hip
@@ -11,21 +11,21 @@
 template <bool COUNT, bool PROF, bool OCC, bool LDS_TABLES>
 __device__ __forceinline__ void trace_lanes(const Scene &sc, const SubRoot *subs, const Inst *insts, PassEps eps,
                                             uint32_t *stack, CoopLds coop, Ray r, uint32_t kind, float T, float remain,
-                                            uint32_t seg, bool active, float4 *res, uint32_t gi) {
+                                            uint32_t seg, bool active, float4 *res, uint32_t gi, float *jvis) {
     for (;;) {
-        const float t_max = !active ? __builtin_nanf("") : kind != Q_CLOSEST ? vis_bound(remain) : 1e10f;
+        const float t_max = !active ? __builtin_nanf("") : (kind & kKindMask) != Q_CLOSEST ? vis_bound(remain) : 1e10f;
         const Hit h = (LDS_TABLES && !COUNT)
                           ? trace_core_flat<PROF, OCC>(sc, subs, insts, r, eps, stack, WB, t_max, coop, remain)
                           : trace_core_tab<COUNT, PROF, true, OCC, true>(sc, subs, insts, r, eps, stack, WB, t_max, coop,
                                                                          false, remain);
-        if (active && end_query(sc, subs, insts, eps, h, r, kind, T, remain, seg, res, gi)) active = false;
+        if (active && end_query(sc, subs, insts, eps, h, r, kind, T, remain, seg, res, gi, jvis)) active = false;
         if (wballot(active) == 0ull) break;
     }
 }
 template <bool COUNT, bool PROF, bool OCC, bool LDS_TABLES>
 __device__ __forceinline__ void trace_batch(const Scene &sc, const SubRoot *subs, const Inst *insts, PassEps eps,
                                             uint32_t *stack, CoopLds coop, float4 *res_all, const float4 *rays_all,
-                                            uint32_t gbase, uint32_t i, bool active) {
+                                            uint32_t gbase, uint32_t i, bool active, float *jvis) {
     const uint32_t gi = gbase + i;
     float4 a = make_float4(0.0f, 0.0f, 0.0f, 0.0f), b = make_float4(0.0f, 0.0f, 1.0f, 0.0f);
     if (active) {
@@ -33,7 +33,7 @@
         b = rays_all[2u * gi + 1u];
     }
     trace_lanes<COUNT, PROF, OCC, LDS_TABLES>(sc, subs, insts, eps, stack, coop, Ray{mk(a.x, a.y, a.z), mk(b.x, b.y, b.z)},
-                                              asu(b.w), 1.0f, a.w, 0u, active, res_all, gi);
+                                              asu(b.w), 1.0f, a.w, 0u, active, res_all, gi, jvis);
 }
 
 template <bool COUNT, int WAVES, bool PROF = false, bool LDS_TABLES = true, bool OCC = false>
@@ -63,7 +63,7 @@
     for (uint32_t i0 = 0u; i0 < n; i0 += WB) {
         const uint32_t i = i0 + threadIdx.x;
         trace_batch<COUNT, PROF, OCC, LDS_TABLES>(sc, subs, insts, eps, stack, coop, res_buf(w, round), w.rays,
-                                                   j * w.ray_stride, i, i < n);
+                                                   j * w.ray_stride, i, i < n, w.jvis);
     }
 }
 
@@ -669,7 +669,8 @@
                 res[2u * slot] = make_float4(0.0f, Le.x, Le.y, Le.z);
             }
         }
-        trace_batch<false, false, false, true>(sc, T.subs, T.insts, eps, stack, coop, res, rays, 0u, slot, active);
+        trace_batch<false, false, false, true>(sc, T.subs, T.insts, eps, stack, coop, res, rays, 0u, slot, active,
+                                               nullptr);
         if (active) {
             if (s.phase == 0u) {
                 const Hit h = get_hit(res, slot);
diff --git a/pathtracerdemo_amd/csrc/ptx_wave_common.h b/pathtracerdemo_amd/csrc/ptx_wave_common.h
--- a/pathtracerdemo_amd/csrc/ptx_wave_common.h
+++ b/pathtracerdemo_amd/csrc/ptx_wave_common.h
@@ -9,6 +9,8 @@
 #define LOGIC_WAVES 4
 #endif
 enum : uint32_t { Q_CLOSEST = 0u, Q_VIS = 1u, Q_OCC = 2u };
+constexpr uint32_t kKindMask = 3u;
+__device__ __forceinline__ uint32_t kind_plane_slot(uint32_t slot) { return (slot + 1u) << 2; }
 
 __device__ __forceinline__ uint32_t wave_scan(uint32_t v, uint32_t &total) { return wave_excl_sum(v, total); }
 __device__ __forceinline__ uint32_t wave_alloc(uint32_t *lds_ctr, uint32_t n) {
@@ -26,16 +28,12 @@
     uint32_t rbase;
     float4 *rays, *res_out;
     const float4 *res_in;
-    uint32_t out_sel;
     uint32_t *act_out;
     const uint32_t *act_in;
     uint32_t n_in;
     uint32_t *l_ray, *l_act;
 };
-__device__ __forceinline__ uint32_t res_sel(const WaveBufs &w, uint32_t round) {
-    return w.nres == 3u ? round % 3u : round & 1u;
-}
-__device__ __forceinline__ float4 *res_buf(const WaveBufs &w, uint32_t round) { return w.res[res_sel(w, round)]; }
+__device__ __forceinline__ float4 *res_buf(const WaveBufs &w, uint32_t round) { return w.res[round & 1u]; }
 __device__ __forceinline__ uint32_t seg_n_in(const WaveBufs &w, uint32_t round) {
     return round ? w.cnt[(2u * (round - 1u)) * w.cnt_stride + w.seg_phys + w.seg_base + blockIdx.x] : 0u;
 }
@@ -48,7 +46,6 @@
     g.rays = w.rays;
     g.res_out = res_buf(w, round);
     g.res_in = round ? res_buf(w, round - 1u) : w.res[1];
-    g.out_sel = res_sel(w, round);
     g.act_out = w.act[round & 1u] + (size_t)g.pj * w.act_stride;
     g.act_in = w.act[(round + 1u) & 1u] + (size_t)g.pj * w.act_stride;
     g.n_in = seg_n_in(w, round);
@@ -123,8 +120,9 @@
 #define PTX_LDS_TRANS 1
 #endif
 __device__ __forceinline__ bool end_query(const Scene &sc, const SubRoot *subs, const Inst *insts, PassEps eps, Hit h,
-                                          Ray &ray, uint32_t kind, float &T, float &remain, uint32_t &seg, float4 *res,
-                                          uint32_t gi) {
+                                          Ray &ray, uint32_t kword, float &T, float &remain, uint32_t &seg, float4 *res,
+                                          uint32_t gi, float *jvis) {
+    const uint32_t kind = kword & kKindMask;
     if (kind == Q_CLOSEST) {
         if (h.valid) complete_hit(sc, ray, eps, h, insts);
         const uint32_t enc = ((h.valid ? 1u : 0u) << 31) | (h.s.inst << 16) | h.s.mat;
@@ -149,7 +147,8 @@
         }
     }
     if (out < 0.0f) return false;
-    res[2u * gi].x = out;
+    if (kword >> 2) jvis[(kword >> 2) - 1u] = out;
+    else res[2u * gi].x = out;
     return true;
 }
 __device__ __forceinline__ f3 x0_of(const Scene &sc, uint32_t x, uint32_t y) {
```

Measured after the change: 589.5 Msamples/s, median of 6. Within noise of the previous version (+0.8%).
